# RTCartist/Neuromorphic-Spatiotemporal-Optical-Flow

Measured on AMD Instinct MI355X. Metric: 1080p frame-pairs/sec (Farneback, HIP), higher is better.
Workload: dtype f32

## Files before the change

### include/nsof.h

```cpp
#ifndef NSOF_H
#define NSOF_H

#include <stddef.h>
#include <stdint.h>

#ifdef __cplusplus
extern "C" {
#endif

#define NSOF_ABI_VERSION 3

typedef enum nsof_status {
    NSOF_OK = 0,
    NSOF_EINVAL = -1,
    NSOF_ESHAPE = -2,
    NSOF_EDEVICE = -3,
    NSOF_ENOMEM = -4,
    NSOF_EUNSUPPORTED = -5
} nsof_status;

typedef struct nsof_ctx nsof_ctx;

int nsof_create(int device, nsof_ctx** out);
void nsof_destroy(nsof_ctx* ctx);
const char* nsof_last_error(const nsof_ctx* ctx);
int nsof_abi_version(void);
int nsof_set_stream(nsof_ctx* ctx, void* hip_stream);
int nsof_synchronize(nsof_ctx* ctx);
enum { NSOF_OPT_POLYEXP_F32 = 1, NSOF_OPT_EXACT_ROWSUMS = 2, NSOF_OPT_ROW_BANDS = 3, NSOF_OPT_PYR_FMA = 4,
       NSOF_OPT_SMALL_BATCH_JOBS = 5, NSOF_OPT_DEBUG_FAULT = 100 };
int nsof_set_option(nsof_ctx* ctx, int option, int value);
int nsof_get_option(const nsof_ctx* ctx, int option, int* value);

enum { NSOF_USE_INITIAL_FLOW = 4, NSOF_FARNEBACK_GAUSSIAN = 256 };

typedef enum nsof_pixel_type {
    NSOF_PIXEL_U8 = 0,
    NSOF_PIXEL_F32 = 1,
    NSOF_PIXEL_U16 = 2,
    NSOF_PIXEL_S16 = 3,
} nsof_pixel_type;

int nsof_farneback_px(nsof_ctx* ctx, int pixel_type,
                      const void* prev, ptrdiff_t prev_stride,
                      const void* next, ptrdiff_t next_stride,
                      int width, int height,
                      float* flow, ptrdiff_t flow_stride,
                      double pyr_scale, int levels, int winsize, int iterations,
                      int poly_n, double poly_sigma, int flags);
int nsof_farneback_u8(nsof_ctx* ctx,
                      const uint8_t* prev, ptrdiff_t prev_stride,
                      const uint8_t* next, ptrdiff_t next_stride,
                      int width, int height,
                      float* flow, ptrdiff_t flow_stride,
                      double pyr_scale, int levels, int winsize, int iterations,
                      int poly_n, double poly_sigma, int flags);
int nsof_farneback_f32(nsof_ctx* ctx,
                       const float* prev, ptrdiff_t prev_stride,
                       const float* next, ptrdiff_t next_stride,
                       int width, int height,
                       float* flow, ptrdiff_t flow_stride,
                       double pyr_scale, int levels, int winsize, int iterations,
                       int poly_n, double poly_sigma, int flags);

int nsof_farneback_px_batch_dev(nsof_ctx* ctx, int pixel_type, int n_pairs,
                                const void* d_prev, const void* d_next,
                                ptrdiff_t row_stride, ptrdiff_t pair_stride,
                                int width, int height, float* d_flow,
                                double pyr_scale, int levels, int winsize, int iterations,
                                int poly_n, double poly_sigma, int flags);
int nsof_farneback_u8_batch_dev(nsof_ctx* ctx, int n_pairs,
                                const uint8_t* d_prev, const uint8_t* d_next,
                                ptrdiff_t row_stride, ptrdiff_t pair_stride,
                                int width, int height, float* d_flow,
                                double pyr_scale, int levels, int winsize, int iterations,
                                int poly_n, double poly_sigma, int flags);
int nsof_farneback_f32_batch_dev(nsof_ctx* ctx, int n_pairs,
                                 const float* d_prev, const float* d_next,
                                 ptrdiff_t row_stride, ptrdiff_t pair_stride,
                                 int width, int height, float* d_flow,
                                 double pyr_scale, int levels, int winsize, int iterations,
                                 int poly_n, double poly_sigma, int flags);

int nsof_farneback_px_sequence_dev(nsof_ctx* ctx, int pixel_type, int n_frames, const void* d_frames,
                                   ptrdiff_t row_stride, ptrdiff_t frame_stride,
                                   int width, int height, float* d_flow,
                                   double pyr_scale, int levels, int winsize, int iterations,
                                   int poly_n, double poly_sigma, int flags);
int nsof_farneback_u8_sequence_dev(nsof_ctx* ctx, int n_frames, const uint8_t* d_frames,
                                   ptrdiff_t row_stride, ptrdiff_t frame_stride,
                                   int width, int height, float* d_flow,
                                   double pyr_scale, int levels, int winsize, int iterations,
                                   int poly_n, double poly_sigma, int flags);
int nsof_farneback_f32_sequence_dev(nsof_ctx* ctx, int n_frames, const float* d_frames,
                                    ptrdiff_t row_stride, ptrdiff_t frame_stride,
                                    int width, int height, float* d_flow,
                                    double pyr_scale, int levels, int winsize, int iterations,
                                    int poly_n, double poly_sigma, int flags);

typedef struct nsof_pair_desc_px {
    const void* prev;
    ptrdiff_t prev_stride;
    const void* next;
    ptrdiff_t next_stride;
    int width, height;
    float* flow;
    ptrdiff_t flow_stride;
} nsof_pair_desc_px;
typedef struct nsof_pair_desc {
    const uint8_t* prev;
    ptrdiff_t prev_stride;
    const uint8_t* next;
    ptrdiff_t next_stride;
    int width, height;
    float* flow;
    ptrdiff_t flow_stride;
} nsof_pair_desc;
typedef struct nsof_pair_desc_f32 {
    const float* prev;
    ptrdiff_t prev_stride;
    const float* next;
    ptrdiff_t next_stride;
    int width, height;
    float* flow;
    ptrdiff_t flow_stride;
} nsof_pair_desc_f32;

int nsof_farneback_px_batch(nsof_ctx* ctx, int pixel_type, int n_pairs, const nsof_pair_desc_px* pairs,
                            double pyr_scale, int levels, int winsize, int iterations,
                            int poly_n, double poly_sigma, int flags);
int nsof_farneback_u8_batch(nsof_ctx* ctx, int n_pairs, const nsof_pair_desc* pairs,
                            double pyr_scale, int levels, int winsize, int iterations,
                            int poly_n, double poly_sigma, int flags);
int nsof_farneback_f32_batch(nsof_ctx* ctx, int n_pairs, const nsof_pair_desc_f32* pairs,
                             double pyr_scale, int levels, int winsize, int iterations,
                             int poly_n, double poly_sigma, int flags);

int nsof_farneback_px_batch_desc_dev(nsof_ctx* ctx, int pixel_type, int n_pairs, const nsof_pair_desc_px* pairs,
                                     double pyr_scale, int levels, int winsize, int iterations,
                                     int poly_n, double poly_sigma, int flags);
int nsof_farneback_u8_batch_desc_dev(nsof_ctx* ctx, int n_pairs, const nsof_pair_desc* pairs,
                                     double pyr_scale, int levels, int winsize, int iterations,
                                     int poly_n, double poly_sigma, int flags);
int nsof_farneback_f32_batch_desc_dev(nsof_ctx* ctx, int n_pairs, const nsof_pair_desc_f32* pairs,
                                      double pyr_scale, int levels, int winsize, int iterations,
                                      int poly_n, double poly_sigma, int flags);

int nsof_farneback_px_roi_sequence_dev(nsof_ctx* ctx, int pixel_type, int n_frames, const void* d_frames,
                                       ptrdiff_t row_stride, ptrdiff_t frame_stride, int width, int height,
                                       const int32_t* d_counts, const int32_t* d_rects, int max_rects, float* d_flows,
                                       double pyr_scale, int levels, int winsize, int iterations, int poly_n,
                                       double poly_sigma, int flags, int gate_frame, long long* n_calls,
                                       long long* n_pixels);
int nsof_farneback_u8_roi_sequence_dev(nsof_ctx* ctx, int n_frames, const uint8_t* d_frames, ptrdiff_t row_stride,
                                       ptrdiff_t frame_stride, int width, int height, const int32_t* d_counts,
                                       const int32_t* d_rects, int max_rects, float* d_flows, double pyr_scale, int levels,
                                       int winsize, int iterations, int poly_n, double poly_sigma, int flags,
                                       int gate_frame, long long* n_calls, long long* n_pixels);
int nsof_farneback_f32_roi_sequence_dev(nsof_ctx* ctx, int n_frames, const float* d_frames, ptrdiff_t row_stride,
                                        ptrdiff_t frame_stride, int width, int height, const int32_t* d_counts,
                                        const int32_t* d_rects, int max_rects, float* d_flows, double pyr_scale, int levels,
                                        int winsize, int iterations, int poly_n, double poly_sigma, int flags,
                                        int gate_frame, long long* n_calls, long long* n_pixels);
void* nsof_host_alloc(size_t bytes);
void nsof_host_free(void* p);

int nsof_farneback_effective_levels(int width, int height, double pyr_scale, int levels);
int nsof_farneback_level_size(int width, int height, double pyr_scale, int level,
                              int* level_width, int* level_height, int* blur_ksize, double* blur_sigma);

int nsof_stage_pyr_level_px(nsof_ctx* ctx, int pixel_type, int n_img, const void* d_src, ptrdiff_t row_stride,
                            ptrdiff_t img_stride, int width, int height, double pyr_scale, int level, float* d_out);
int nsof_stage_pyr_level(nsof_ctx* ctx, int n_img, const uint8_t* d_src, ptrdiff_t row_stride,
                         ptrdiff_t img_stride, int width, int height, double pyr_scale, int level, float* d_out);
int nsof_stage_pyr_level_f32(nsof_ctx* ctx, int n_img, const float* d_src, ptrdiff_t row_stride,
                             ptrdiff_t img_stride, int width, int height, double pyr_scale, int level, float* d_out);
int nsof_stage_polyexp(nsof_ctx* ctx, int n_img, const float* d_img, int width, int height,
                       int poly_n, double poly_sigma, float* d_R);
int nsof_stage_recip(nsof_ctx* ctx, long long n, const double* d_x, double* d_out, double* d_ieee);
int nsof_stage_update_matrices(nsof_ctx* ctx, int n_pairs, const float* d_R, const float* d_flow,
                               int width, int height, float* d_M);
int nsof_stage_blur_solve(nsof_ctx* ctx, int n_pairs, const float* d_M, int width, int height,
                          int winsize, float* d_flow);
int nsof_stage_gauss_blur_solve(nsof_ctx* ctx, int n_pairs, const float* d_M, int width, int height,
                                int winsize, float* d_flow);
int nsof_stage_iterate(nsof_ctx* ctx, int n_pairs, const float* d_R, const float* d_flow_in, int width, int height,
                       int winsize, float* d_flow_out);
int nsof_stage_iterate_upsample(nsof_ctx* ctx, int n_pairs, const float* d_R, const float* d_coarse_flow,
                                int src_w, int src_h, int width, int height, int winsize, double pyr_scale,
                                float* d_flow_out);
int nsof_stage_flow_upsample(nsof_ctx* ctx, int n_pairs, const float* d_src, int src_w, int src_h,
                             float* d_dst, int dst_w, int dst_h, double pyr_scale);

typedef enum nsof_kernel_id {
    NSOF_K_PREP = 0,
    NSOF_K_POLYEXP = 1,
    NSOF_K_UPSAMPLE = 2,
    NSOF_K_UPDMAT = 3,
    NSOF_K_BLUR = 4,
    NSOF_K_ACCUM = 5,
    NSOF_K_ITERATE = 6,
    NSOF_K_SEGMENT = 7,
    NSOF_K_MORPH = 8,
    NSOF_K_REMAP = 9,
    NSOF_K_SSIM = 10,
    NSOF_K_COUNT = 11
} nsof_kernel_id;
int nsof_prof_enable(nsof_ctx* ctx, unsigned mask);
int nsof_prof_collect(nsof_ctx* ctx, int kernel_id, double* total_ms, long long* launches);
const char* nsof_kernel_name(int kernel_id);

typedef struct nsof_accum nsof_accum;

int nsof_accum_create(nsof_ctx* ctx, int height, int width, int scheme, int polarity_split,
                      float active_v, float silent_v, nsof_accum** out);
typedef struct nsof_accum_params {
    double alphaoff, alphaon, voff, von, koff, kon, son, soff, bon, boff, Ron, Roff, wini;
    double dt;
    int64_t refractory_us;
} nsof_accum_params;
void nsof_accum_default_params(nsof_accum_params* out);
int nsof_accum_create_p(nsof_ctx* ctx, int height, int width, int scheme, int polarity_split, float active_v, float silent_v,
                        const nsof_accum_params* params, nsof_accum** out);
int nsof_accum_get_params(const nsof_accum* acc, nsof_accum_params* out);
enum {
    NSOF_ACCUM_KEY_ALPHAOFF = 0, NSOF_ACCUM_KEY_ALPHAON, NSOF_ACCUM_KEY_VOFF, NSOF_ACCUM_KEY_VON, NSOF_ACCUM_KEY_KOFF,
    NSOF_ACCUM_KEY_KON, NSOF_ACCUM_KEY_SON, NSOF_ACCUM_KEY_SOFF, NSOF_ACCUM_KEY_BON, NSOF_ACCUM_KEY_BOFF, NSOF_ACCUM_KEY_RON,
    NSOF_ACCUM_KEY_ROFF, NSOF_ACCUM_KEY_WINI, NSOF_ACCUM_KEY_COUNT
};
int nsof_accum_set_param_maps(nsof_accum* acc, int n_maps, const int* keys, const float* const* maps);
int nsof_accum_read_param_map(nsof_accum* acc, int key, float* out);
int nsof_accum_param_map_mask(const nsof_accum* acc, unsigned* mask);
void nsof_accum_destroy(nsof_accum* acc);
int nsof_accum_set_dense(nsof_accum* acc, int force_dense);
int nsof_accum_set_event_threshold(nsof_accum* acc, int theta);
int nsof_accum_get_event_threshold(const nsof_accum* acc, int* theta);
int nsof_accum_reset(nsof_accum* acc);
int nsof_accum_step_events(nsof_accum* acc, const int16_t* x, const int16_t* y, const int8_t* p,
                           const int64_t* t, const int64_t* slice_bounds, int64_t n_slices,
                           int64_t snap_every);
int nsof_accum_set_events(nsof_accum* acc, const int16_t* x, const int16_t* y, const int8_t* p,
                          const int64_t* t, const int64_t* slice_bounds, int64_t n_slices);
int nsof_accum_run(nsof_accum* acc, int64_t first_slice, int64_t n_slices, int64_t snap_every);
int nsof_accum_set_slice_times(nsof_accum* acc, const int64_t* t_first, const int64_t* t_last, int64_t n_slices);
enum { NSOF_SURFACE_CURRENT = 0, NSOF_SURFACE_STATE = 1 };
int nsof_accum_surface_u8_dev(nsof_accum* acc, int which, int mode, uint8_t* d_out, ptrdiff_t row_stride);
int nsof_accum_surface_f32_dev(nsof_accum* acc, int which, int mode, float* d_out, ptrdiff_t row_stride_bytes);
int nsof_accum_run_surface(nsof_accum* a, int64_t first_slice, int64_t n_slices, int which, int mode, uint8_t* d_out,
                           ptrdiff_t row_stride);
int nsof_accum_run_frames(nsof_accum* acc, int64_t first_slice, int64_t n_frames, int64_t every, int which, int mode,
                          uint8_t* d_frames, ptrdiff_t row_stride, ptrdiff_t frame_stride);
int nsof_accum_set_frames_path(nsof_accum* acc, int path);
int nsof_accum_read_state(nsof_accum* acc, int which, float* w_out, int64_t* next_ok_out, int64_t* slice_counter);
int nsof_accum_write_state(nsof_accum* acc, int which, const float* w_in, const int64_t* next_ok_in,
                           int64_t slice_counter);
int nsof_accum_update_state_dev(nsof_ctx* ctx, const float* d_w, const float* d_V, float* d_out, size_t n);
int nsof_accum_update_state_p_dev(nsof_ctx* ctx, const nsof_accum_params* params, const float* d_w, const float* d_V,
                                  float* d_out, size_t n);
int nsof_accum_bincount_2d(nsof_ctx* ctx, const int16_t* x, const int16_t* y, size_t n, int height, int width,
                           int32_t* counts_out);
int nsof_accum_resistance_dev(nsof_ctx* ctx, const float* d_w, float* d_out, size_t n);
int nsof_accum_resistance_p_dev(nsof_ctx* ctx, const nsof_accum_params* params, const float* d_w, float* d_out, size_t n);
int nsof_accum_read_w(nsof_accum* acc, int which, float* w_out);
int nsof_accum_read_resistance(nsof_accum* acc, int which, float* r_out);
int64_t nsof_accum_snapshot_count(const nsof_accum* acc);
int nsof_accum_read_snapshots(nsof_accum* acc, int which, float* out, int64_t max_count);
int nsof_accum_block_current(nsof_accum* acc, int which, int64_t snapshot, int memsize, double v_ds, double* out);
int nsof_accum_block_current_dev(nsof_accum* acc, int which, int64_t snapshot, int memsize, double v_ds, double* d_out);
int nsof_accum_frames_f64(nsof_ctx* ctx, const double* imgs, int n_frames, int height, int width, double dt,
                          int n_sub_steps, double th1, double th2, double* w_out, double* res_out);
int nsof_accum_frames_f64_p(nsof_ctx* ctx, const double* imgs, int n_frames, int height, int width, double dt,
                            int n_sub_steps, double th1, double th2, const nsof_accum_params* params, double* w_out,
                            double* res_out);
int nsof_accum_frames_f64_dev(nsof_ctx* ctx, const double* d_imgs, int n_frames, int height, int width, double dt,
                              int n_sub_steps, double th1, double th2, double v_ds, double* d_w, double* d_res,
                              double* d_current);
int nsof_accum_frames_f64_p_dev(nsof_ctx* ctx, const double* d_imgs, int n_frames, int height, int width, double dt,
                                int n_sub_steps, double th1, double th2, double v_ds, const nsof_accum_params* params,
                                double* d_w, double* d_res, double* d_current);
int nsof_accum_frames_f64_maps_dev(nsof_ctx* ctx, const double* d_imgs, int n_frames, int height, int width, double dt,
                                   int n_sub_steps, double th1, double th2, double v_ds, const nsof_accum_params* params,
                                   int n_trials, int n_maps, const int* keys, const double* const* planes,
                                   const int* plane_trials, double* d_w, double* d_res, double* d_current);
int nsof_accum_frames_f64_maps(nsof_ctx* ctx, const double* imgs, int n_frames, int height, int width, double dt,
                               int n_sub_steps, double th1, double th2, const nsof_accum_params* params, int n_trials,
                               int n_maps, const int* keys, const double* const* planes, const int* plane_trials,
                               double* w_out, double* res_out);
int nsof_accum_trials_dev(nsof_ctx* ctx, int height, int width, int scheme, int polarity_split, float active_v, float silent_v,
                          const nsof_accum_params* params, int theta, const int16_t* x, const int16_t* y, const int8_t* p,
                          const int64_t* t, const int64_t* slice_bounds, int64_t n_slices, int64_t snap_every, int memsize,
                          double v_ds, int n_trials, int n_maps, const int* keys, const float* const* planes,
                          const int* plane_trials, float* d_w, float* d_resistance, double* d_block_current);
int nsof_frames_compress_u8_dev(nsof_ctx* ctx, int n_frames, const uint8_t* d_frames, ptrdiff_t row_stride,
                                ptrdiff_t frame_stride, int width, int height, int out_w, int out_h, const double* wts_y,
                                const int32_t* ind_y, int taps_y, const double* wts_x, const int32_t* ind_x, int taps_x,
                                double* d_out);
int nsof_lanczos3_contributions(int in_len, int out_len, double* wts, int32_t* ind, int cap_taps, int* taps);
int64_t nsof_accum_slice_bounds(const int64_t* t, int64_t n, int64_t slice_us, int64_t* idx, int64_t cap);

int nsof_roi_from_surface(const double* current, int rows, int cols, int frame_w, int frame_h, int memsize, int thres,
                          int extend_left, int extend_right, int extend_upper, int extend_lower, int connectivity,
                          int flag, int* rects, int max_rects);

int nsof_roi_from_surface_dev(nsof_ctx* ctx, const double* d_current, int n_maps, size_t map_stride, int rows, int cols,
                              int frame_w, int frame_h, int memsize, int thres, int extend_left, int extend_right,
                              int extend_upper, int extend_lower, int connectivity, int flag, int max_rects, int* d_counts,
                              int* d_rects, unsigned char* d_gray);
int nsof_gate_stats_dev(nsof_ctx* ctx, const double* d_current, const double* d_nominal, int n_trials, int n_frames, int rows,
                        int cols, int thres, int* d_counts, int* d_flips);

enum { NSOF_MORPH_RECT = 0, NSOF_MORPH_CROSS = 1, NSOF_MORPH_ELLIPSE = 2 };
enum { NSOF_MORPH_ERODE = 0, NSOF_MORPH_DILATE = 1 };
int nsof_structuring_element(int shape, int kw, int kh, uint8_t* out);
int nsof_morph_binary_u8_dev(nsof_ctx* ctx, int op, const uint8_t* d_src, ptrdiff_t src_stride, int width,
                             int height, const uint8_t* elem, int kw, int kh, int anchor_x, int anchor_y,
                             int iterations, uint8_t* d_dst, ptrdiff_t dst_stride);
int nsof_motion_mask_dev(nsof_ctx* ctx, const float* d_flow, ptrdiff_t flow_stride_floats, int width, int height,
                         double thresh, int ksize, int iterations, uint8_t* d_mask, ptrdiff_t mask_stride);
int nsof_motion_mask_sequence_dev(nsof_ctx* ctx, int n_pairs, const float* d_flows, int width, int height,
                                  const int32_t* box_counts, const int32_t* boxes, double thresh, int ksize,
                                  int iterations, uint8_t* d_masks);
int nsof_pixel_accuracy_u8_batch_dev(nsof_ctx* ctx, int n, const uint8_t* d_masks, const uint8_t* d_gt,
                                     ptrdiff_t gt_row_stride, ptrdiff_t gt_frame_stride, int width, int height,
                                     double* d_out);
int nsof_motion_mask(nsof_ctx* ctx, const float* flow, ptrdiff_t flow_stride_bytes, int width, int height,
                     double thresh, int ksize, int iterations, uint8_t* mask, ptrdiff_t mask_stride);

enum { NSOF_BORDER_CONSTANT = 0, NSOF_BORDER_REPLICATE = 1 };
int nsof_gray_u8_dev(nsof_ctx* ctx, const uint8_t* d_src, ptrdiff_t src_stride, int width, int height, int bgr_weights,
                     uint8_t* d_dst, ptrdiff_t dst_stride);
int nsof_remap_linear_u8_dev(nsof_ctx* ctx, const uint8_t* d_src, ptrdiff_t src_stride, int src_w, int src_h,
                             int channels, const float* d_map_x, ptrdiff_t map_x_stride_floats,
                             const float* d_map_y, ptrdiff_t map_y_stride_floats, int dst_w, int dst_h,
                             int border_mode, int border_value, uint8_t* d_dst, ptrdiff_t dst_stride);
int nsof_predict_warp_u8_dev(nsof_ctx* ctx, const uint8_t* d_frame, ptrdiff_t frame_stride, int width, int height,
                             int channels, const float* d_flow, ptrdiff_t flow_stride_floats, int sign,
                             int x0, int y0, int x1, int y1, int border_mode, uint8_t* d_out, ptrdiff_t out_stride);
int nsof_predict_warp_u8(nsof_ctx* ctx, const uint8_t* frame, ptrdiff_t frame_stride, int width, int height,
                         int channels, const float* flow_crop, ptrdiff_t flow_stride_bytes, int sign,
                         int x0, int y0, int x1, int y1, int border_mode, uint8_t* out, ptrdiff_t out_stride);
int nsof_ssim_u8_dev(nsof_ctx* ctx, const uint8_t* d_a, ptrdiff_t a_stride, int a_pixel_step, const uint8_t* d_b,
                     ptrdiff_t b_stride, int b_pixel_step, int width, int height, double data_range,
                     double* ssim_out);
int nsof_ssim_u8(nsof_ctx* ctx, const uint8_t* a, ptrdiff_t a_stride, int a_pixel_step, const uint8_t* b,
                 ptrdiff_t b_stride, int b_pixel_step, int width, int height, double data_range, double* ssim_out);
int nsof_predict_sequence_u8_dev(nsof_ctx* ctx, int n_pairs, const uint8_t* d_frames, ptrdiff_t row_stride,
                                 ptrdiff_t frame_stride, int width, int height, const float* d_flows, int sign,
                                 const int32_t* d_counts, const int32_t* d_rects, int n_maps, int max_rects,
                                 int gate_frame, int merge_padding, int border_mode, uint8_t* d_out);
int nsof_ssim_u8_batch_dev(nsof_ctx* ctx, int n, const uint8_t* d_a, ptrdiff_t a_stride, ptrdiff_t a_item_stride,
                           int a_pixel_step, const uint8_t* d_b, ptrdiff_t b_stride, ptrdiff_t b_item_stride,
                           int b_pixel_step, int width, int height, double data_range, double* d_out);
int nsof_flow_to_image_dev(nsof_ctx* ctx, int n, const float* d_flows, ptrdiff_t row_stride_floats,
                           ptrdiff_t item_stride_floats, int width, int height, int sign, double clip_flow,
                           double max_flow, int convert_to_bgr, uint8_t* d_out, ptrdiff_t out_row_stride,
                           ptrdiff_t out_item_stride, float* d_norms);

#ifdef __cplusplus
}
#endif
#endif
```

### neuromorphic-spatiotemporal-optical-flow_amd/csrc/farneback_driver.hip

```cpp
#include <cstdlib>
#include <cstring>

#include "nsof_internal.h"

struct Carve {
    std::vector<size_t> offI, offR;
    size_t szI = 0, szR = 0, szS = 0, szM = 0, szV = 0;
    char* base = nullptr;
    size_t total() const { return szI + szR + szS + szM + szV; }
    float* level_I(int k) const { return (float*)(base + offI[k]); }
    float* level_R(int k) const { return (float*)(base + szI + offR[k]); }
    float* S() const { return (float*)(base + szI + szR); }
    float* M() const { return (float*)(base + szI + szR + szS); }
    double* V() const { return (double*)(base + szI + szR + szS + szM); }
};
static Carve farneback_carve(size_t B, bool sequence, int width, int height, double pyr_scale, int L, bool lat,
                             nsof_iter_form form)
{
    Carve c;
    c.offI.assign(L + 1, 0);
    c.offR.assign(L + 1, 0);
    const size_t n0 = (size_t)width * height;
    const size_t n_img = sequence ? B + 1 : 2 * B;
    for (int k = 0; k <= (lat ? L : 0); k++) {
        int wk, hk;
        nsof_farneback_level_size(width, height, pyr_scale, k, &wk, &hk, nullptr, nullptr);
        c.offI[k] = c.szI;
        c.offR[k] = c.szR;
        c.szI += align_up(n_img * (size_t)wk * hk * 4, 256);
        c.szR += align_up(n_img * 5 * (size_t)wk * hk * 4, 256);
    }
    c.szS = align_up(B * n0 * 8, 256);
    const bool M = form != NSOF_ITER_FAST && form != NSOF_ITER_EXACT;
    const bool V = form == NSOF_ITER_UNFUSED_EXACT || form == NSOF_ITER_EXACT_LAT;
    c.szM = M ? align_up(B * 5 * n0 * 4, 256) : 0;
    c.szV = V ? align_up(B * 5 * n0 * 8, 256) : 0;
    return c;
}

struct Run {
    nsof_ctx* ctx;
    const nsof_fb_frames& f;
    const nsof_fb_params& p;
    int L;
    nsof_iter_form form;
    bool lat;
    Carve cv;
    size_t B, n_img;
    int arrays, n_first;
    nsof_poly_taps ptaps;
    float* Ifused[4] = {nullptr, nullptr, nullptr, nullptr};
};

static int level_images(const Run& r, int k, int wk, int hk, const nsof_blur_taps& bt)
{
    const nsof_fb_frames& f = r.f;
    float* Rk = r.cv.level_R(k);
    if (k >= 1 && k <= 3 && r.Ifused[k]) return nsof_launch_polyexp(r.ctx, (int)r.n_img, r.Ifused[k], wk, hk, r.ptaps, Rk);
    if (k == 0 && nsof_level0_from_frames(r.ctx, f.src, bt) && f.width >= 2 && f.height >= 2 && wk == f.width && hk == f.height)
        return nsof_launch_polyexp_frames(r.ctx, (int)r.n_img, f.prev, r.arrays == 1 ? f.prev : f.next, r.n_first, f.row_stride,
                                          f.pair_stride, f.width, f.height, r.ptaps, bt.k[1], bt.k[2], Rk, f.src);
    float* I = r.cv.level_I(k);
    for (int i = 0; i < r.arrays; i++)
        if (int rc = nsof_launch_prep(r.ctx, r.n_first, i == 0 ? f.prev : f.next, f.row_stride, f.pair_stride, f.width, f.height, wk,
                                      hk, bt, I + (size_t)i * r.B * wk * hk, f.src))
            return rc;
    return nsof_launch_polyexp(r.ctx, (int)r.n_img, I, wk, hk, r.ptaps, Rk);
}

static int side_stream_images(const Run& r)
{
    nsof_ctx* ctx = r.ctx;
    const int L = r.L;
    if (!ctx->side) NSOF_HIP(ctx, hipStreamCreateWithFlags(&ctx->side, hipStreamNonBlocking));
    while (ctx->ov_events.size() < (size_t)(L + 2)) {
        hipEvent_t ev;
        NSOF_HIP(ctx, hipEventCreateWithFlags(&ev, hipEventDisableTiming));
        ctx->ov_events.push_back(ev);
    }
    const hipStream_t mainS = ctx->stream, sideS = ctx->side;
    struct Restore { nsof_ctx* cx; hipStream_t saved; ~Restore() { cx->stream = saved; } } restore{ctx, mainS};
    NSOF_HIP(ctx, hipEventRecord(ctx->ov_events[L + 1], mainS));
    NSOF_HIP(ctx, hipStreamWaitEvent(sideS, ctx->ov_events[L + 1], 0));
    for (int k = L; k >= 0; k--) {
        int wk, hk;
        nsof_blur_taps bt;
        if (int rc = nsof_level_geom(ctx, r.f.width, r.f.height, r.p.pyr_scale, k, &wk, &hk, &bt)) return rc;
        ctx->stream = k == L ? mainS : sideS;
        if (int rc = level_images(r, k, wk, hk, bt)) return rc;
        if (k < L) NSOF_HIP(ctx, hipEventRecord(ctx->ov_events[k], sideS));
    }
    return NSOF_OK;
}

static int three_level_images(Run& r)
{
    const nsof_fb_frames& f = r.f;
    nsof_blur_taps bt3[3];
    size_t nk3[3];
    for (int k = 1; k <= 3; k++) {
        int wk, hk;
        if (nsof_level_geom(nullptr, f.width, f.height, r.p.pyr_scale, k, &wk, &hk, &bt3[k - 1]) != 0 ||
            wk * (1 << k) != f.width || hk * (1 << k) != f.height)
            return NSOF_OK;
        nk3[k - 1] = (size_t)wk * hk;
    }
    float* dI = r.cv.level_I(0);
    float* I3[3] = {dI, dI + r.n_img * nk3[0], dI + r.n_img * (nk3[0] + nk3[1])};
    int rc = NSOF_OK;
    for (size_t i = 0; i < (size_t)r.arrays && rc == NSOF_OK; i++) {
        float* I3i[3] = {I3[0] + i * r.B * nk3[0], I3[1] + i * r.B * nk3[1], I3[2] + i * r.B * nk3[2]};
        rc = nsof_launch_prep_decim3(r.ctx, r.n_first, i == 0 ? f.prev : f.next, f.row_stride, f.pair_stride, f.width, f.height, bt3,
                                     I3i, f.src);
    }
    if (rc == NSOF_OK)
        for (int k = 1; k <= 3; k++) r.Ifused[k] = I3[k - 1];
    return rc == NSOF_EUNSUPPORTED ? NSOF_OK : rc;
}

static int iterate_level(const Run& r, int k, int wk, int hk, float* const fb[2], int* cur)
{
    nsof_ctx* ctx = r.ctx;
    const int n_pairs = r.f.n_pairs, winsize = r.p.winsize;
    const size_t nk = (size_t)wk * hk;
    const float* R0 = r.cv.level_R(k);
    const float* R1 = R0 + (r.f.sequence ? (size_t)1 : r.B) * 5 * nk;
    float* dM = r.cv.M();
    double* dV = r.cv.V();
    for (int it = 0; it < r.p.iterations; it++) {
        int rc;
        if (nsof_form_fused(r.form)) {
            float* in = fb[*cur];
            float* out = fb[*cur ^= 1];
            if (r.form == NSOF_ITER_EXACT_LAT) rc = nsof_launch_iterate_lat(ctx, n_pairs, R0, R1, 5 * nk, in, out, wk, hk, winsize, dM, dV);
            else if (r.form == NSOF_ITER_EXACT) rc = nsof_launch_iterate_x(ctx, n_pairs, R0, R1, 5 * nk, in, out, wk, hk, winsize);
            else rc = nsof_launch_iterate(ctx, n_pairs, R0, R1, 5 * nk, in, out, wk, hk, winsize);
        } else {
            float* flow = fb[*cur];
            if ((rc = nsof_launch_update_matrices(ctx, n_pairs, R0, R1, 5 * nk, flow, wk, hk, dM))) return rc;
            if (r.form == NSOF_ITER_UNFUSED_GAUSS) rc = nsof_launch_gauss_blur_solve(ctx, n_pairs, dM, wk, hk, winsize, flow);
            else if (r.form == NSOF_ITER_UNFUSED_EXACT) rc = nsof_launch_blur_solve_exact(ctx, n_pairs, dM, wk, hk, winsize, dV, flow);
            else rc = nsof_launch_blur_solve(ctx, n_pairs, dM, wk, hk, winsize, flow);
        }
        if (rc) return rc;
    }
    return NSOF_OK;
}

static int run_levels(Run& r, float* d_flow)
{
    nsof_ctx* ctx = r.ctx;
    const nsof_fb_frames& f = r.f;
    const int L = r.L, iterations = r.p.iterations;
    int rc = nsof_host_poly_taps(r.p.poly_n, r.p.poly_sigma, &r.ptaps);
    if (rc) return nsof_set_error(ctx, rc, "poly taps");
    if ((rc = ctx->ws.reserve(ctx, r.cv.total()))) return rc;
    r.cv.base = (char*)ctx->ws.p;
    float* const fb[2] = {d_flow, r.cv.S()};
    const int flips = nsof_form_fused(r.form) ? L * (1 + iterations) + iterations : L;
    int cur = flips & 1;

    const hipStream_t mainS = ctx->stream;
    if (r.lat) rc = side_stream_images(r);
    else if (L == 3) rc = three_level_images(r);
    if (rc) return rc;

    int pw = 0, ph = 0;
    for (int k = L; k >= 0; k--) {
        int wk, hk;
        nsof_blur_taps btaps;
        if ((rc = nsof_level_geom(ctx, f.width, f.height, r.p.pyr_scale, k, &wk, &hk, &btaps))) return rc;
        if (k == L) {
            NSOF_HIP(ctx, hipMemsetAsync(fb[cur], 0, r.B * wk * hk * 8, mainS));
        } else {
            if ((rc = nsof_launch_flow_upsample(ctx, f.n_pairs, fb[cur], pw, ph, fb[cur ^ 1], wk, hk, (float)(1. / r.p.pyr_scale))))
                return rc;
            cur ^= 1;
        }
        if (!r.lat) {
            if ((rc = level_images(r, k, wk, hk, btaps))) return rc;
        } else if (k < L) {
            NSOF_HIP(ctx, hipStreamWaitEvent(mainS, ctx->ov_events[k], 0));
        }
        if ((rc = iterate_level(r, k, wk, hk, fb, &cur))) return rc;
        pw = wk;
        ph = hk;
    }
    if (fb[cur] != d_flow)
        NSOF_HIP(ctx, hipMemcpyAsync(d_flow, fb[cur], r.B * f.width * f.height * 8, hipMemcpyDeviceToDevice, mainS));
    return NSOF_OK;
}

static int pairs_per_run(Run& r, size_t* fit)
{
    nsof_ctx* ctx = r.ctx;
    auto carve = [&](size_t b) { return farneback_carve(b, r.f.sequence, r.f.width, r.f.height, r.p.pyr_scale, r.L, r.lat, r.form); };
    size_t n = (size_t)r.f.n_pairs;
    if (r.form == NSOF_ITER_UNFUSED_EXACT && n > 64) n = 64;
    r.cv = carve(n);
    if (r.cv.total() > ctx->ws.cap) {
        size_t free_b = 0, total_b = 0;
        NSOF_HIP(ctx, hipMemGetInfo(&free_b, &total_b));
        const size_t budget = (size_t)((double)(free_b + ctx->ws.cap) * 0.92);
        size_t lo = 0, hi = n;
        while (lo < hi) {
            const size_t mid = (lo + hi + 1) / 2;
            if (carve(mid).total() <= budget) lo = mid;
            else hi = mid - 1;
        }
        n = lo;
    }
    if (const char* e = getenv("NSOF_MAX_PAIRS")) {
        const long v = atol(e);
        if (v >= 1 && (size_t)v < n) n = (size_t)v;
    }
    if (n < 1) n = 1;
    if (n > 32767) n = 32767;
    *fit = n;
    return NSOF_OK;
}

int nsof_farneback_core(nsof_ctx* ctx, const nsof_fb_frames& frames, float* d_flow, const nsof_fb_params& p)
{
    if (!ctx) return NSOF_EINVAL;
    nsof_fb_frames f = frames;
    if (f.sequence) f.next = f.prev;
    if (!f.prev || !f.next || !d_flow || f.n_pairs < 1) return nsof_set_error(ctx, NSOF_EINVAL, "null buffer or n_pairs<1");
    int rc = nsof_check_farneback_params(ctx, f.width, f.height, p);
    if (rc) return rc;
    if (!nsof_row_stride_holds(f.row_stride, f.width, f.src))
        return nsof_set_error(ctx, NSOF_EINVAL, "row_stride < width * %d", nsof_src_bytes(f.src));
    NSOF_HIP(ctx, hipSetDevice(ctx->device));
    const nsof_iter_form form = nsof_iterate_form(ctx, p.winsize, f.width, f.height, p.iterations,
                                                  f.n_pairs * nsof_iterate_jobs(f.width, f.height), p.flags);
    if (form == NSOF_ITER_UNFUSED_EXACT && f.sequence) {
        f.sequence = false;
        f.next = f.prev + f.pair_stride;
    }
    const int L = nsof_farneback_effective_levels(f.width, f.height, p.pyr_scale, p.levels);
    Run r{ctx, f, p, L, form, form == NSOF_ITER_EXACT_LAT && L >= 1};
    size_t fit;
    if ((rc = pairs_per_run(r, &fit))) return rc;
    if ((size_t)f.n_pairs > fit) {
        nsof_fb_frames c = f;
        for (int i = 0; i < f.n_pairs; i += (int)fit) {
            c.n_pairs = f.n_pairs - i < (int)fit ? f.n_pairs - i : (int)fit;
            c.prev = f.prev + (ptrdiff_t)i * f.pair_stride;
            c.next = f.next + (ptrdiff_t)i * f.pair_stride;
            if ((rc = nsof_farneback_core(ctx, c, d_flow + (size_t)i * f.width * f.height * 2, p))) return rc;
        }
        return NSOF_OK;
    }
    r.B = (size_t)f.n_pairs;
    r.n_img = f.sequence ? r.B + 1 : 2 * r.B;
    r.arrays = f.sequence || f.next == f.prev + (ptrdiff_t)f.n_pairs * f.pair_stride ? 1 : 2;
    r.n_first = r.arrays == 1 ? (int)r.n_img : f.n_pairs;
    return run_levels(r, d_flow);
}

extern "C" int nsof_farneback_px_batch_dev(nsof_ctx* ctx, int pixel_type, int n_pairs, const void* d_prev, const void* d_next,
                                           ptrdiff_t row_stride, ptrdiff_t pair_stride, int width, int height, float* d_flow,
                                           double pyr_scale, int levels, int winsize, int iterations, int poly_n,
                                           double poly_sigma, int flags)
{
    if (int rc = nsof_check_typed(ctx, pixel_type)) return rc;
    if (!d_prev || !d_next || !d_flow) return nsof_set_error(ctx, NSOF_EINVAL, "null buffer");
    int rc = nsof_check_frame_layout(ctx, pixel_type, d_prev, row_stride, pair_stride, width, "d_prev");
    if (rc == NSOF_OK) rc = nsof_check_frame_layout(ctx, pixel_type, d_next, row_stride, pair_stride, width, "d_next");
    if (rc) return rc;
    return nsof_farneback_core(ctx, {false, n_pairs, (const uint8_t*)d_prev, (const uint8_t*)d_next, row_stride, pair_stride, width,
                                     height, pixel_type},
                               d_flow, {pyr_scale, levels, winsize, iterations, poly_n, poly_sigma, flags});
}

extern "C" int nsof_farneback_px_sequence_dev(nsof_ctx* ctx, int pixel_type, int n_frames, const void* d_frames,
                                              ptrdiff_t row_stride, ptrdiff_t frame_stride, int width, int height,
                                              float* d_flow, double pyr_scale, int levels, int winsize, int iterations,
                                              int poly_n, double poly_sigma, int flags)
{
    if (int rc = nsof_check_typed(ctx, pixel_type)) return rc;
    if (n_frames < 2) return nsof_set_error(ctx, NSOF_EINVAL, "a sequence needs at least 2 frames");
    if (!d_frames || !d_flow) return nsof_set_error(ctx, NSOF_EINVAL, "null buffer");
    if (int rc = nsof_check_frame_layout(ctx, pixel_type, d_frames, row_stride, frame_stride, width, "d_frames")) return rc;
    return nsof_farneback_core(ctx, {true, n_frames - 1, (const uint8_t*)d_frames, nullptr, row_stride, frame_stride, width, height,
                                     pixel_type},
                               d_flow, {pyr_scale, levels, winsize, iterations, poly_n, poly_sigma, flags});
}

extern "C" int nsof_farneback_px(nsof_ctx* ctx, int src, const void* prev, ptrdiff_t prev_stride, const void* next,
                                 ptrdiff_t next_stride, int width, int height, float* flow, ptrdiff_t flow_stride,
                                 double pyr_scale, int levels, int winsize, int iterations, int poly_n,
                                 double poly_sigma, int flags)
{
    if (int rc = nsof_check_typed(ctx, src)) return rc;
    const nsof_fb_params p{pyr_scale, levels, winsize, iterations, poly_n, poly_sigma, flags};
    if (!prev || !next || !flow) return nsof_set_error(ctx, NSOF_EINVAL, "null image pointer");
    int rc = nsof_check_farneback_params(ctx, width, height, p);
    if (rc) return rc;
    if ((rc = nsof_check_frame_layout(ctx, src, prev, prev_stride, 0, width, "prev")) ||
        (rc = nsof_check_frame_layout(ctx, src, next, next_stride, 0, width, "next")))
        return rc;
    if (flow_stride < (ptrdiff_t)(width * 8)) return nsof_set_error(ctx, NSOF_EINVAL, "flow_stride < width*8");
    NSOF_HIP(ctx, hipSetDevice(ctx->device));
    const size_t n0 = (size_t)width * height, pitch = (size_t)width * nsof_src_bytes(src);
    const size_t szU = align_up(pitch * height, 256), szF = align_up(n0 * 8, 256);
    if ((rc = ctx->stage.reserve(ctx, 2 * szU + szF)) || (rc = ctx->hstage.reserve(ctx, 2 * szU + szF))) return rc;
    char* hP = (char*)ctx->hstage.p;
    char* hN = hP + szU;
    float* hF = (float*)(hN + szU);
    uint8_t* dP = (uint8_t*)ctx->stage.p;
    uint8_t* dN = dP + szU;
    float* dFl = (float*)(dN + szU);
    const bool in_dense = prev_stride == (ptrdiff_t)pitch && next_stride == (ptrdiff_t)pitch;
    const bool out_dense = flow_stride == (ptrdiff_t)width * 8;
    if (in_dense) {
        NSOF_HIP(ctx, hipMemcpyAsync(dP, prev, pitch * height, hipMemcpyHostToDevice, ctx->stream));
        NSOF_HIP(ctx, hipMemcpyAsync(dN, next, pitch * height, hipMemcpyHostToDevice, ctx->stream));
    } else {
        for (int y = 0; y < height; y++) {
            memcpy(hP + (size_t)y * pitch, (const char*)prev + (ptrdiff_t)y * prev_stride, pitch);
            memcpy(hN + (size_t)y * pitch, (const char*)next + (ptrdiff_t)y * next_stride, pitch);
        }
        NSOF_HIP(ctx, hipMemcpyAsync(dP, hP, 2 * szU, hipMemcpyHostToDevice, ctx->stream));
    }
    if ((rc = nsof_farneback_core(ctx, {false, 1, dP, dN, (ptrdiff_t)pitch, (ptrdiff_t)szU, width, height, src}, dFl, p))) return rc;
    NSOF_HIP(ctx, hipMemcpyAsync(out_dense ? flow : hF, dFl, n0 * 8, hipMemcpyDeviceToHost, ctx->stream));
    if ((rc = nsof_stream_sync_checked(ctx))) return rc;
    if (!out_dense)
        for (int y = 0; y < height; y++)
            memcpy((char*)flow + (ptrdiff_t)y * flow_stride, hF + (size_t)y * width * 2, (size_t)width * 8);
    return NSOF_OK;
}

extern "C" int nsof_farneback_u8(nsof_ctx* ctx, const uint8_t* prev, ptrdiff_t prev_stride, const uint8_t* next,
                                 ptrdiff_t next_stride, int width, int height, float* flow, ptrdiff_t flow_stride,
                                 double pyr_scale, int levels, int winsize, int iterations, int poly_n,
                                 double poly_sigma, int flags)
{
    return nsof_farneback_px(ctx, NSOF_PIXEL_U8, prev, prev_stride, next, next_stride, width, height, flow, flow_stride,
                             pyr_scale, levels, winsize, iterations, poly_n, poly_sigma, flags);
}

extern "C" int nsof_farneback_f32(nsof_ctx* ctx, const float* prev, ptrdiff_t prev_stride, const float* next,
                                  ptrdiff_t next_stride, int width, int height, float* flow, ptrdiff_t flow_stride,
                                  double pyr_scale, int levels, int winsize, int iterations, int poly_n,
                                  double poly_sigma, int flags)
{
    return nsof_farneback_px(ctx, NSOF_PIXEL_F32, prev, prev_stride, next, next_stride, width, height, flow, flow_stride,
                             pyr_scale, levels, winsize, iterations, poly_n, poly_sigma, flags);
}

extern "C" int nsof_farneback_u8_batch_dev(nsof_ctx* ctx, int n_pairs, const uint8_t* d_prev, const uint8_t* d_next,
                                           ptrdiff_t row_stride, ptrdiff_t pair_stride, int width, int height,
                                           float* d_flow, double pyr_scale, int levels, int winsize, int iterations,
                                           int poly_n, double poly_sigma, int flags)
{
    return nsof_farneback_px_batch_dev(ctx, NSOF_PIXEL_U8, n_pairs, d_prev, d_next, row_stride, pair_stride, width, height,
                                       d_flow, pyr_scale, levels, winsize, iterations, poly_n, poly_sigma, flags);
}

extern "C" int nsof_farneback_f32_batch_dev(nsof_ctx* ctx, int n_pairs, const float* d_prev, const float* d_next,
                                            ptrdiff_t row_stride, ptrdiff_t pair_stride, int width, int height,
                                            float* d_flow, double pyr_scale, int levels, int winsize, int iterations,
                                            int poly_n, double poly_sigma, int flags)
{
    return nsof_farneback_px_batch_dev(ctx, NSOF_PIXEL_F32, n_pairs, d_prev, d_next, row_stride, pair_stride, width, height,
                                       d_flow, pyr_scale, levels, winsize, iterations, poly_n, poly_sigma, flags);
}

extern "C" int nsof_farneback_u8_sequence_dev(nsof_ctx* ctx, int n_frames, const uint8_t* d_frames,
                                              ptrdiff_t row_stride, ptrdiff_t frame_stride, int width, int height,
                                              float* d_flow, double pyr_scale, int levels, int winsize,
                                              int iterations, int poly_n, double poly_sigma, int flags)
{
    return nsof_farneback_px_sequence_dev(ctx, NSOF_PIXEL_U8, n_frames, d_frames, row_stride, frame_stride, width, height,
                                          d_flow, pyr_scale, levels, winsize, iterations, poly_n, poly_sigma, flags);
}

extern "C" int nsof_farneback_f32_sequence_dev(nsof_ctx* ctx, int n_frames, const float* d_frames,
                                               ptrdiff_t row_stride, ptrdiff_t frame_stride, int width, int height,
                                               float* d_flow, double pyr_scale, int levels, int winsize,
                                               int iterations, int poly_n, double poly_sigma, int flags)
{
    return nsof_farneback_px_sequence_dev(ctx, NSOF_PIXEL_F32, n_frames, d_frames, row_stride, frame_stride, width, height,
                                          d_flow, pyr_scale, levels, winsize, iterations, poly_n, poly_sigma, flags);
}
```

### neuromorphic-spatiotemporal-optical-flow_amd/csrc/farneback_iterate_x.hip

```cpp
#include "iterate_common.h"

namespace {

typedef __attribute__((address_space(1))) unsigned long long gu64;
typedef __attribute__((address_space(1))) unsigned gu32;
typedef __attribute__((address_space(3))) int lds_int;

__device__ __forceinline__ unsigned xcc_id() { return __builtin_amdgcn_s_getreg(20 | (0 << 6) | (3 << 11)) & 7u; }

template <int MH>
struct XGeom {
    static constexpr int COLS = 208, NCW = 3, RB = 4;
    static constexpr int RL = 2 * MH + 1 + 2 * RB;
    static constexpr int HALO = 2 * MH + 1;
    static constexpr int SW = NCW * 64;
    static_assert(SW + HALO <= COLS && SW % 8 == 0, "strip geometry");
    static constexpr int NB = COLS / 64, REM = COLS % 64;
    static_assert(REM == 16, "the remainder wave maps 4 rows x 16 columns onto its 64 lanes");
    static constexpr int SEG0 = 96, SEG1 = SW - SEG0;
    static_assert(SEG0 % 8 == 0 && SEG1 % 8 == 0 && SEG0 >= SEG1 && SEG1 > 0, "segments: whole 8-column blocks, the left one not shorter");
    static constexpr int SVW = SW + 2;
    static constexpr int WAVES = NCW + 1 + 2 * NB + 1 + 1;
    static constexpr int THREADS = 64 * WAVES;
    static constexpr int CQ = 1, IOQ = 1;
    static constexpr size_t SV1_BYTES = sizeof(double) * 4 * 5 * SVW;
    static constexpr size_t SV_BYTES = 2 * SV1_BYTES;
    static constexpr size_t VI_BYTES = sizeof(double) * 2 * 4 * 5 * MH;
    static constexpr size_t JOB_BYTES = 16;
    static constexpr size_t CB_BYTES = sizeof(double) * 2 * 2 * 20;
    static constexpr size_t RING4_BYTES = sizeof(float) * 4 * RL * COLS, RING1_BYTES = sizeof(float) * RL * COLS;
    static constexpr size_t SMEM = SV_BYTES + VI_BYTES + JOB_BYTES + CB_BYTES + RING4_BYTES + RING1_BYTES;
};

struct XRing {
    float4* q;
    float* c;
    int cols;
    __device__ __forceinline__ void put(int slot, int col, const float (&M)[5]) const
    {
        q[slot * cols + col] = make_float4(M[0], M[1], M[2], M[3]);
        c[slot * cols + col] = M[4];
    }
    __device__ __forceinline__ void get(int slot, int col, float (&M)[5]) const
    {
        const float4 v = q[slot * cols + col];
        M[0] = v.x; M[1] = v.y; M[2] = v.z; M[3] = v.w;
        M[4] = c[slot * cols + col];
    }
};

constexpr unsigned X_SPIN_LIMIT = 1u << 21;

template <int MH>
__device__ __forceinline__ void x_produce(RowIn& in, float2& dd, float2& fl, const XRing& ring, const Planes& R0,
                                          const Planes& R1, const FlowSrc& F, int W, int H, int xc, int col, int i)
{
    constexpr int RL = XGeom<MH>::RL;
    float Mn[5];
    matrix_from(in, dd.x, dd.y, xc, min(i, H - 1), W, H, Mn);
    ring.put((i + MH + 1) % RL, col, Mn);
    issue_row(in, R0, R1, W, H, xc, min(i + 8, H - 1), fl);
    dd = fl;
    fl = F.fetch(min(i + 16, H - 1));
}

template <int MH>
__device__ __forceinline__ void x_rows_above(const XRing& ring, const Planes& R0, const Planes& R1, const FlowSrc& F,
                                             int W, int H, int xc, int col)
{
    float2 fl[MH];
#pragma unroll
    for (int i = 0; i < MH; i++) fl[i] = F.fetch(min(i, H - 1));
    constexpr int GRP = 4;
#pragma unroll
    for (int g0 = 0; g0 < MH; g0 += GRP) {
        RowIn t[GRP];
#pragma unroll
        for (int k = 0; k < GRP; k++)
            if (g0 + k < MH) issue_row(t[k], R0, R1, W, H, xc, min(g0 + k, H - 1), fl[g0 + k]);
#pragma unroll
        for (int k = 0; k < GRP; k++)
            if (g0 + k < MH) {
                float Mi[5];
                matrix_from(t[k], fl[g0 + k].x, fl[g0 + k].y, xc, min(g0 + k, H - 1), W, H, Mi);
                if (g0 + k == 0) {
#pragma unroll
                    for (int j = 0; j <= MH + 1; j++) ring.put(j, col, Mi);
                } else {
                    ring.put(g0 + k + MH + 1, col, Mi);
                }
            }
    }
}

template <int MH, int GP>
__device__ __forceinline__ void x_producer_loop(const XRing& ring, const Planes& R0, const Planes& R1,
                                                const FlowSrc& F, int W, int H, int xc, int col, int nimg)
{
    if constexpr (GP == 0) x_rows_above<MH>(ring, R0, R1, F, W, H, xc, col);
    RowIn in[2][2];
    float2 dd[2][2], fl[2][2];
#pragma unroll
    for (int ts = 0; ts < 2; ts++)
#pragma unroll
        for (int rr = 0; rr < 2; rr++) {
            const int r = min(4 * ts + MH + 2 * GP + rr, H - 1);
            dd[ts][rr] = F.fetch(r);
            issue_row(in[ts][rr], R0, R1, W, H, xc, r, dd[ts][rr]);
        }
#pragma unroll
    for (int ts = 0; ts < 2; ts++)
#pragma unroll
        for (int rr = 0; rr < 2; rr++) fl[ts][rr] = F.fetch(min(4 * (ts + 2) + MH + 2 * GP + rr, H - 1));
    auto step = [&](auto tsc, int t) {
        constexpr int TS = decltype(tsc)::value;
        x_produce<MH>(in[TS][0], dd[TS][0], fl[TS][0], ring, R0, R1, F, W, H, xc, col, 4 * t + MH + 2 * GP);
        x_produce<MH>(in[TS][1], dd[TS][1], fl[TS][1], ring, R0, R1, F, W, H, xc, col, 4 * t + MH + 2 * GP + 1);
    };
    step(std::integral_constant<int, 0>{}, 0);
    __syncthreads();
    step(std::integral_constant<int, 1>{}, 1);
    __syncthreads();
    int t = 0;
    for (; t < nimg; t += 2) {
        step(std::integral_constant<int, 0>{}, t + 2);
        __syncthreads();
        step(std::integral_constant<int, 1>{}, t + 3);
        __syncthreads();
    }
    if (t == nimg) {
        step(std::integral_constant<int, 0>{}, t + 2);
        __syncthreads();
    }
}

template <int MH, int Q0, int NQ>
__device__ __forceinline__ void x_solve_rows(const double* sv, volatile lds_int* flag, float2* Fout, size_t fpitch, int W, int H,
                                             int x0, int nimg, double scale, int lane, int t)
{
    using G = XGeom<MH>;
    constexpr int SVW = G::SVW, NBLK = G::SW / 64;
    double g[NBLK][NQ][5];
    int us[NBLK];
#pragma unroll
    for (int b = 0; b < NBLK; b++) {
        const int col = b * 64 + lane;
        const int u = t - 1 - (col >= G::SEG0 ? 1 : 0);
        us[b] = (u >= 0 && u < nimg && x0 + col < W) ? u : -1;
        const double* p = sv + (u & 1) * (G::SV1_BYTES / sizeof(double)) + col;
#pragma unroll
        for (int q = 0; q < NQ; q++)
#pragma unroll
            for (int c = 0; c < 5; c++) g[b][q][c] = p[((q + Q0) * 5 + c) * SVW];
    }
    asm volatile("s_waitcnt lgkmcnt(0)" ::: "memory");
    if (lane == 0) *flag = t + 1;
#pragma unroll
    for (int b = 0; b < NBLK; b++) {
        if (us[b] < 0) continue;
        const int x = x0 + b * 64 + lane;
#pragma unroll
        for (int q = 0; q < NQ; q++) {
            const int yo = 4 * us[b] + q + Q0;
            const float2 o = nsof_flow_solve(g[b][q][0], g[b][q][1], g[b][q][2], g[b][q][3], g[b][q][4], scale);
            if (yo < H) nsof_store_stream2(reinterpret_cast<float*>(Fout + (size_t)yo * fpitch + x), o.x, o.y);
        }
    }
}

template <int MH>
__device__ __forceinline__ void x_remainder_loop(const XRing& ring, double* cb, const Planes& R0, const Planes& R1,
                                                 const FlowSrc& F, int W, int H, int xc, int col, int r, int nimg,
                                                 gu64* cin, gu64* cout, unsigned epoch, gu32* err, const double* sv,
                                                 volatile lds_int* ioflag, float2* Fout, size_t fpitch, int x0, double scale)
{
    const int lane = threadIdx.x & 63;
    const bool io = lane < 20;
    const int l = io ? lane : 0;
    unsigned long long g0 = 0, g1 = 0;
    auto carry_load = [&](int s) {
        const gu64* q = cin + 40 * s + 2 * l;
        asm volatile("global_load_dwordx2 %0, %2, off sc1\n\tglobal_load_dwordx2 %1, %2, off offset:8 sc1"
                     : "=&v"(g0), "=&v"(g1) : "v"(q) : "memory");
    };
    auto fetch_issue = [&](int s) {
        if (!cin || !io) return;
        carry_load(s);
    };
    bool dead = false;
    auto fetch_finish = [&](int s) {
        if (!cin || !io) return;
        asm volatile("s_waitcnt vmcnt(9)" : "+v"(g0), "+v"(g1) : : "memory");
        for (unsigned spins = 0; !dead; spins++) {
            if (__all((unsigned)(g0 >> 32) == epoch && (unsigned)(g1 >> 32) == epoch)) break;
            if (spins > X_SPIN_LIMIT ||
                ((spins & 255u) == 255u && __hip_atomic_load(err, __ATOMIC_RELAXED, __HIP_MEMORY_SCOPE_AGENT) != 0u)) {
                if (lane == 0) __hip_atomic_fetch_or(err, 1u, __ATOMIC_RELAXED, __HIP_MEMORY_SCOPE_AGENT);
                dead = true;
                break;
            }
            __builtin_amdgcn_s_sleep(8);
            carry_load(s);
            asm volatile("s_waitcnt vmcnt(0)" : "+v"(g0), "+v"(g1) : : "memory");
        }
        cb[40 + (s & 1) * 20 + l] = __hiloint2double((int)(unsigned)g1, (int)(unsigned)g0);
    };
    auto publish = [&](int s) {
        if (!cout || !io) return;
        const double S = cb[(s & 1) * 20 + l];
        const unsigned long long tag = (unsigned long long)epoch << 32;
        __hip_atomic_store(cout + 40 * s + 2 * l, tag | (unsigned)__double2loint(S), __ATOMIC_RELAXED, __HIP_MEMORY_SCOPE_AGENT);
        __hip_atomic_store(cout + 40 * s + 2 * l + 1, tag | (unsigned)__double2hiint(S), __ATOMIC_RELAXED, __HIP_MEMORY_SCOPE_AGENT);
    };
    if (r == 0) x_rows_above<MH>(ring, R0, R1, F, W, H, xc, col);
    RowIn in[2];
    float2 dd[2], fl[2];
#pragma unroll
    for (int ts = 0; ts < 2; ts++) {
        const int y = min(4 * ts + MH + r, H - 1);
        dd[ts] = F.fetch(y);
        issue_row(in[ts], R0, R1, W, H, xc, y, dd[ts]);
    }
#pragma unroll
    for (int ts = 0; ts < 2; ts++) fl[ts] = F.fetch(min(4 * (ts + 2) + MH + r, H - 1));
    x_produce<MH>(in[0], dd[0], fl[0], ring, R0, R1, F, W, H, xc, col, MH + r);
    __syncthreads();
    fetch_issue(0);
    x_produce<MH>(in[1], dd[1], fl[1], ring, R0, R1, F, W, H, xc, col, 4 + MH + r);
    fetch_finish(0);
    __syncthreads();
    auto window = [&](auto tsc, int t) {
        constexpr int TS = decltype(tsc)::value;
        if (t >= 2) publish(t - 2);
        if (t + 1 < nimg) fetch_issue(t + 1);
        x_produce<MH>(in[TS], dd[TS], fl[TS], ring, R0, R1, F, W, H, xc, col, 4 * (t + 2) + MH + r);
        x_solve_rows<MH, XGeom<MH>::CQ, XGeom<MH>::IOQ>(sv, ioflag, Fout, fpitch, W, H, x0, nimg, scale, lane, t);
        if (t + 1 < nimg) fetch_finish(t + 1);
        __syncthreads();
    };
    int t = 0;
    for (; t < nimg; t += 2) {
        window(std::integral_constant<int, 0>{}, t);
        window(std::integral_constant<int, 1>{}, t + 1);
    }
    if (t == nimg) window(std::integral_constant<int, 0>{}, t);
    publish(nimg - 1);
    x_solve_rows<MH, XGeom<MH>::CQ, XGeom<MH>::IOQ>(sv, ioflag, Fout, fpitch, W, H, x0, nimg, scale, lane, nimg + 1);
}

template <int MH>
__device__ __forceinline__ void x_consumer_loop(const XRing& ring, double* sv, double* vinit, volatile lds_int* sflag, float2* Fout,
                                                size_t fpitch, int W, int H, int x0, int j, int nimg, double scale, bool strip0)
{
    using G = XGeom<MH>;
    constexpr int RL = G::RL, SVW = G::SVW, HALO = G::HALO;
    const int rb = j, ra = j + HALO;
    const int vik = j == 0 ? 0 : j - MH - 1;
    const bool vi_thread = strip0 && (j == 0 || (j >= MH + 2 && j <= 2 * MH));
    __syncthreads();
    double va[5], vb[5];
    {
        float a0[5], b0[5];
        ring.get(MH + 1, ra, a0);
        ring.get(MH + 1, rb, b0);
#pragma unroll
        for (int c = 0; c < 5; c++) {
            va[c] = (double)(a0[c] * (float)(MH + 2));
            vb[c] = (double)(b0[c] * (float)(MH + 2));
        }
#pragma unroll
        for (int i = 1; i < MH; i++) {
            ring.get(i + MH + 1, ra, a0);
            ring.get(i + MH + 1, rb, b0);
#pragma unroll
            for (int c = 0; c < 5; c++) {
                va[c] += (double)a0[c];
                vb[c] += (double)b0[c];
            }
        }
    }
    int slot_new = (2 * MH + 1) % RL;
    int slot_old = 0;
    const int x = x0 + j;
    const int lag = j >= G::SEG0 ? 1 : 0;
    double D[2][4][5];
    auto column_sums = [&](auto pc, int s) {
        constexpr int P = decltype(pc)::value;
#pragma unroll
        for (int q = 0; q < 4; q++) {
            float na[5], oa[5], nb[5], ob[5];
            ring.get(slot_new, ra, na);
            ring.get(slot_old, ra, oa);
            ring.get(slot_new, rb, nb);
            ring.get(slot_old, rb, ob);
#pragma unroll
            for (int c = 0; c < 5; c++) {
                const float da = na[c] - oa[c];
                const float db = nb[c] - ob[c];
                va[c] += (double)da;
                vb[c] += (double)db;
                D[P][q][c] = va[c] - vb[c];
            }
            if (vi_thread) {
#pragma unroll
                for (int c = 0; c < 5; c++) vinit[(((s & 1) * 4 + q) * 5 + c) * MH + vik] = vb[c];
            }
            slot_new = slot_new + 1 == RL ? 0 : slot_new + 1;
            slot_old = slot_old + 1 == RL ? 0 : slot_old + 1;
        }
    };
    auto publish = [&](auto pc, int p) {
        constexpr int P = decltype(pc)::value;
        if (p < 0 || p >= nimg) return;
        double* svj = sv + (p & 1) * (G::SV1_BYTES / sizeof(double)) + j;
#pragma unroll
        for (int q = 0; q < 4; q++)
#pragma unroll
            for (int c = 0; c < 5; c++) svj[(q * 5 + c) * SVW] = D[P][q][c];
    };
    column_sums(std::integral_constant<int, 0>{}, 0);
    if (!lag) publish(std::integral_constant<int, 0>{}, 0);
    __syncthreads();
    auto window = [&](auto pc, int t) {
        constexpr int P = decltype(pc)::value;
        const int u = t - 1 - lag;
        if (u >= 0 && u < nimg && x < W) {
            const double* svj = sv + (u & 1) * (G::SV1_BYTES / sizeof(double)) + j;
#pragma unroll
            for (int q = 0; q < G::CQ; q++) {
                const int yo = 4 * u + q;
                const double* s = svj + q * 5 * SVW;
                const float2 o = nsof_flow_solve(s[0], s[SVW], s[2 * SVW], s[3 * SVW], s[4 * SVW], scale);
                if (yo < H) nsof_store_stream2(reinterpret_cast<float*>(Fout + (size_t)yo * fpitch + x), o.x, o.y);
            }
        }
        if (t == nimg + 1) return;
        if (t + 1 < nimg) column_sums(std::integral_constant<int, P ^ 1>{}, t + 1);
        for (int spin = 0; (sflag[0] < t + 1 || sflag[1] < t + 1) && spin < (1 << 22); spin++)
            __builtin_amdgcn_s_sleep(1);
        if (lag) publish(std::integral_constant<int, P>{}, t);
        else publish(std::integral_constant<int, P ^ 1>{}, t + 1);
        __syncthreads();
    };
    for (int t = 0; t <= nimg + 1; t += 2) {
        window(std::integral_constant<int, 0>{}, t);
        if (t + 1 > nimg + 1) break;
        window(std::integral_constant<int, 1>{}, t + 1);
    }
}

template <int MH>
__device__ __forceinline__ void x_solver_loop(const double* sv, volatile lds_int* sflag, float2* Fout, size_t fpitch, int W, int H,
                                              int x0, int nimg, double scale, int lane)
{
    using G = XGeom<MH>;
    __syncthreads();
    __syncthreads();
    for (int t = 0; t <= nimg + 1; t++) {
        x_solve_rows<MH, G::CQ + G::IOQ, 4 - G::CQ - G::IOQ>(sv, sflag, Fout, fpitch, W, H, x0, nimg, scale, lane, t);
        if (t <= nimg) __syncthreads();
    }
}

template <int MH>
__device__ __forceinline__ void x_scanner_loop(double* sv, const double* vinit, double* cb, bool has_left, int nimg, int ncols,
                                               int lane)
{
    using G = XGeom<MH>;
    constexpr int SVW = G::SVW;
    typedef double d2 __attribute__((ext_vector_type(2)));
    const int seg = lane >= 20 ? 1 : 0;
    const int l = lane < 40 ? lane - 20 * seg : 0;
    double Smid = 0.;
    __syncthreads();
    __builtin_amdgcn_s_setprio(3);
    __syncthreads();
    for (int t = 0; t <= nimg; t++) {
        const int step = t - seg;
        const double Sleft = __shfl(Smid, lane >= 20 ? lane - 20 : lane);
        d2* row = reinterpret_cast<d2*>(sv + (step & 1) * (G::SV1_BYTES / sizeof(double)) + l * SVW + seg * G::SEG0);
        if (lane < 40 && step >= 0 && step < nimg) {
            double S;
            if (seg) {
                S = Sleft;
            } else if (has_left) {
                S = cb[40 + (step & 1) * 20 + l];
            } else {
                const double* vi = vinit + ((step & 1) * 20 + l) * MH;
                S = vi[0] * (double)(MH + 2);
#pragma unroll
                for (int k = 1; k < MH; k++) S += vi[k];
            }
            auto scan_blocks = [&](int b0, int nb) {
                unsigned a = (unsigned)(size_t)(__attribute__((address_space(3))) char*)(row + 4 * b0);
                int nrem = nb - 1;
                asm volatile(
                "ds_read_b128 v[64:67], %[a]\n\t"
                "ds_read_b128 v[68:71], %[a] offset:16\n\t"
                "ds_read_b128 v[72:75], %[a] offset:32\n\t"
                "ds_read_b128 v[76:79], %[a] offset:48\n\t"
                "ds_read_b128 v[80:83], %[a] offset:64\n\t"
                "ds_read_b128 v[84:87], %[a] offset:80\n\t"
                "ds_read_b128 v[88:91], %[a] offset:96\n\t"
                "ds_read_b128 v[92:95], %[a] offset:112\n\t"
                "s_waitcnt lgkmcnt(7)\n\t"
                "v_add_f64 v[64:65], %[S], v[64:65]\n\t"
                "v_add_f64 v[66:67], v[66:67], v[64:65]\n\t"
                "s_waitcnt lgkmcnt(6)\n\t"
                "v_add_f64 v[68:69], v[66:67], v[68:69]\n\t"
                "v_add_f64 v[70:71], v[70:71], v[68:69]\n\t"
                "s_waitcnt lgkmcnt(5)\n\t"
                "v_add_f64 v[72:73], v[70:71], v[72:73]\n\t"
                "v_add_f64 v[74:75], v[74:75], v[72:73]\n\t"
                "s_waitcnt lgkmcnt(4)\n\t"
                "v_add_f64 v[76:77], v[74:75], v[76:77]\n\t"
                "v_add_f64 v[78:79], v[78:79], v[76:77]\n\t"
                "s_nop 1\n\t"
                "ds_write_b128 %[a], v[64:67]\n\t"
                "ds_write_b128 %[a], v[68:71] offset:16\n\t"
                "ds_write_b128 %[a], v[72:75] offset:32\n\t"
                "ds_write_b128 %[a], v[76:79] offset:48\n\t"
                "s_cmp_lt_i32 %[n], 2\n\t"
                "s_cbranch_scc1 .Lxs_tail%=\n"
                ".Lxs_loop%=:\n\t"
                "s_waitcnt lgkmcnt(7)\n\t"
                "v_add_f64 v[80:81], v[78:79], v[80:81]\n\t"
                "ds_read_b128 v[64:67], %[a] offset:128\n\t"
                "ds_read_b128 v[68:71], %[a] offset:144\n\t"
                "ds_read_b128 v[72:75], %[a] offset:160\n\t"
                "ds_read_b128 v[76:79], %[a] offset:176\n\t"
                "v_add_f64 v[82:83], v[82:83], v[80:81]\n\t"
                "s_waitcnt lgkmcnt(10)\n\t"
                "v_add_f64 v[84:85], v[82:83], v[84:85]\n\t"
                "v_add_f64 v[86:87], v[86:87], v[84:85]\n\t"
                "s_waitcnt lgkmcnt(9)\n\t"
                "v_add_f64 v[88:89], v[86:87], v[88:89]\n\t"
                "v_add_f64 v[90:91], v[90:91], v[88:89]\n\t"
                "s_waitcnt lgkmcnt(8)\n\t"
                "v_add_f64 v[92:93], v[90:91], v[92:93]\n\t"
                "v_add_f64 v[94:95], v[94:95], v[92:93]\n\t"
                "s_nop 1\n\t"
                "ds_write_b128 %[a], v[80:83] offset:64\n\t"
                "ds_write_b128 %[a], v[84:87] offset:80\n\t"
                "ds_write_b128 %[a], v[88:91] offset:96\n\t"
                "ds_write_b128 %[a], v[92:95] offset:112\n\t"
                "s_waitcnt lgkmcnt(7)\n\t"
                "v_add_f64 v[64:65], v[94:95], v[64:65]\n\t"
                "ds_read_b128 v[80:83], %[a] offset:192\n\t"
                "ds_read_b128 v[84:87], %[a] offset:208\n\t"
                "ds_read_b128 v[88:91], %[a] offset:224\n\t"
                "ds_read_b128 v[92:95], %[a] offset:240\n\t"
                "v_add_f64 v[66:67], v[66:67], v[64:65]\n\t"
                "s_waitcnt lgkmcnt(10)\n\t"
                "v_add_f64 v[68:69], v[66:67], v[68:69]\n\t"
                "v_add_f64 v[70:71], v[70:71], v[68:69]\n\t"
                "s_waitcnt lgkmcnt(9)\n\t"
                "v_add_f64 v[72:73], v[70:71], v[72:73]\n\t"
                "v_add_f64 v[74:75], v[74:75], v[72:73]\n\t"
                "s_waitcnt lgkmcnt(8)\n\t"
                "v_add_f64 v[76:77], v[74:75], v[76:77]\n\t"
                "v_add_f64 v[78:79], v[78:79], v[76:77]\n\t"
                "s_nop 1\n\t"
                "ds_write_b128 %[a], v[64:67] offset:128\n\t"
                "ds_write_b128 %[a], v[68:71] offset:144\n\t"
                "ds_write_b128 %[a], v[72:75] offset:160\n\t"
                "ds_write_b128 %[a], v[76:79] offset:176\n\t"
                "v_add_u32 %[a], 128, %[a]\n\t"
                "s_sub_i32 %[n], %[n], 2\n\t"
                "s_cmp_ge_i32 %[n], 2\n\t"
                "s_cbranch_scc1 .Lxs_loop%=\n"
                ".Lxs_tail%=:\n\t"
                "s_cmp_lt_i32 %[n], 1\n\t"
                "s_cbranch_scc1 .Lxs_done%=\n\t"
                "s_waitcnt lgkmcnt(4)\n\t"
                "v_add_f64 v[80:81], v[78:79], v[80:81]\n\t"
                "v_add_f64 v[82:83], v[82:83], v[80:81]\n\t"
                "s_waitcnt lgkmcnt(4)\n\t"
                "v_add_f64 v[84:85], v[82:83], v[84:85]\n\t"
                "v_add_f64 v[86:87], v[86:87], v[84:85]\n\t"
                "s_waitcnt lgkmcnt(4)\n\t"
                "v_add_f64 v[88:89], v[86:87], v[88:89]\n\t"
                "v_add_f64 v[90:91], v[90:91], v[88:89]\n\t"
                "s_waitcnt lgkmcnt(4)\n\t"
                "v_add_f64 v[92:93], v[90:91], v[92:93]\n\t"
                "v_add_f64 v[94:95], v[94:95], v[92:93]\n\t"
                "s_nop 1\n\t"
                "ds_write_b128 %[a], v[80:83] offset:64\n\t"
                "ds_write_b128 %[a], v[84:87] offset:80\n\t"
                "ds_write_b128 %[a], v[88:91] offset:96\n\t"
                "ds_write_b128 %[a], v[92:95] offset:112\n\t"
                "v_mov_b64 v[78:79], v[94:95]\n"
                ".Lxs_done%=:\n\t"
                "v_mov_b64 %[S], v[78:79]\n\t"
                "s_waitcnt lgkmcnt(0)\n\t"
                    : [S] "+v"(S), [a] "+v"(a), [n] "+s"(nrem)
                    :
                    : "memory", "scc", "v64", "v65", "v66", "v67", "v68", "v69", "v70", "v71", "v72", "v73", "v74", "v75", "v76", "v77", "v78", "v79", "v80", "v81", "v82", "v83", "v84", "v85", "v86", "v87", "v88", "v89", "v90", "v91", "v92", "v93", "v94", "v95");
            };
            const int nb0 = ncols >> 3, nba = nb0 < G::SEG1 / 8 ? nb0 : G::SEG1 / 8;
            scan_blocks(0, nba);
            if (nb0 > nba && !seg) scan_blocks(nba, nb0 - nba);
            if (seg) cb[(step & 1) * 20 + l] = S;
            else Smid = S;
        }
        __syncthreads();
    }
}

template <int MH, bool HET>
__global__ __launch_bounds__((XGeom<MH>::THREADS)) void k_iterate_x(
    const float* __restrict__ R0b, const float* __restrict__ R1b, size_t pair_stride, const float* __restrict__ flow_in,
    float* __restrict__ flow_out, int W, int H, int block_size, const nsof_het_item* __restrict__ items, int het_final,
    int n, int nstrips, unsigned long long* carry, unsigned* tickets, unsigned epoch, unsigned* err, int fault,
    const unsigned* __restrict__ xjobs)
{
    using G = XGeom<MH>;
    constexpr int SW = G::SW, COLS = G::COLS;
    extern __shared__ __attribute__((aligned(16))) unsigned char smem_x[];
    double* sv = reinterpret_cast<double*>(smem_x);
    double* vinit = reinterpret_cast<double*>(smem_x + G::SV_BYTES);
    int* job = reinterpret_cast<int*>(smem_x + G::SV_BYTES + G::VI_BYTES);
    double* cb = reinterpret_cast<double*>(smem_x + G::SV_BYTES + G::VI_BYTES + G::JOB_BYTES);
    XRing ring;
    ring.q = reinterpret_cast<float4*>(smem_x + G::SV_BYTES + G::VI_BYTES + G::JOB_BYTES + G::CB_BYTES);
    ring.c = reinterpret_cast<float*>(smem_x + G::SV_BYTES + G::VI_BYTES + G::JOB_BYTES + G::CB_BYTES + G::RING4_BYTES);
    ring.cols = COLS;
    const int tid = threadIdx.x;
    if (tid == 0) {
        const unsigned share = HET ? 0u : (unsigned)((n + 7) / 8) * (unsigned)nstrips;
        unsigned k = xcc_id();
        unsigned lim = HET ? xjobs[k] : share;
        unsigned i = __hip_atomic_fetch_add(tickets + 32 * k, 1u, __ATOMIC_RELAXED, __HIP_MEMORY_SCOPE_AGENT);
        if (__hip_atomic_load((gu32*)err, __ATOMIC_RELAXED, __HIP_MEMORY_SCOPE_AGENT) != 0u) i = 0xffffffffu, lim = 0;
        else if (i >= lim) {
            for (unsigned d = 1; d < 8 && i >= lim; d++) {
                k = (k + 1) & 7u;
                if constexpr (HET) lim = xjobs[k];
                i = __hip_atomic_fetch_add(tickets + 32 * k, 1u, __ATOMIC_RELAXED, __HIP_MEMORY_SCOPE_AGENT);
            }
        }
        if constexpr (HET) {
            const unsigned e = i < lim ? xjobs[8u + k * (unsigned)nstrips + i] : 0xffffffffu;
            job[0] = e != 0xffffffffu ? (int)(e >> 8) : -1;
            job[1] = (int)(e & 255u);
        } else {
            job[0] = i < share ? (int)((i / (unsigned)nstrips) * 8u + k) : -1;
            job[1] = (int)(i % (unsigned)nstrips);
        }
        job[2] = job[3] = 0;
    }
    __syncthreads();
    const int pair = job[0], strip = job[1];
    if (pair < 0 || pair >= n) return;
    size_t fpitch = (size_t)W;
    gu64* cbase;
    if constexpr (HET) {
        const nsof_het_item& it = items[pair];
        W = it.wk;
        H = it.hk;
        if (strip * SW >= W) return;
        R0b += it.offR;
        R1b = R0b + 5 * (size_t)W * H;
        pair_stride = 0;
        flow_in += 2 * it.offF;
        cbase = (gu64*)(carry + it.offR / 2);
        if (het_final) {
            flow_out = it.out;
            fpitch = (size_t)it.out_pitch;
        } else {
            flow_out += 2 * it.offF;
            fpitch = (size_t)W;
        }
    } else {
        if (strip * SW >= W) return;
        cbase = (gu64*)(carry + (size_t)pair * nstrips * (size_t)(((H + 3) / 4) * 40));
    }
    const int nimg = (H + 3) / 4;
    const int x0 = strip * SW;
    const size_t plane = (size_t)W * H;
    const size_t poff = HET ? 0 : (size_t)pair * pair_stride;
    const Planes R0 = planes_of(R0b + poff, plane);
    const Planes R1 = planes_of(R1b + poff, plane);
    const int wave = __builtin_amdgcn_readfirstlane(tid >> 6);
    volatile lds_int* sflag = (volatile lds_int*)(job + 2);
    if (wave < G::NCW) {
        float2* Fout = reinterpret_cast<float2*>(flow_out) + (HET ? 0 : (size_t)pair * plane);
        x_consumer_loop<MH>(ring, sv, vinit, sflag, Fout, fpitch, W, H, x0, tid, nimg, 1. / (block_size * block_size), strip == 0);
    } else if (wave == G::WAVES - 1) {
        float2* Fout = reinterpret_cast<float2*>(flow_out) + (HET ? 0 : (size_t)pair * plane);
        x_solver_loop<MH>(sv, sflag, Fout, fpitch, W, H, x0, nimg, 1. / (block_size * block_size), tid & 63);
    } else if (wave == G::NCW) {
        const int ncols = min(G::SEG0, (W - x0 + 7) & ~7);
        x_scanner_loop<MH>(sv, vinit, cb, strip > 0, nimg, ncols, tid & 63);
    } else {
        const int pw = wave - (G::NCW + 1);
        const int lane = tid & 63;
        FlowSrc F;
        F.base = reinterpret_cast<const char*>(flow_in) + (HET ? 0 : (size_t)pair * plane * 8);
        F.W = (unsigned)W;
        const bool is_io = pw == G::NB;
        const int gp = pw < G::NB ? 0 : 1;
        const int blk = pw < G::NB ? pw : pw - G::NB - 1;
        if (is_io) {
            const int col = G::NB * 64 + (lane & 15), r = lane >> 4;
            const int xc = clampi(x0 - MH - 1 + col, 0, W - 1);
            F.xc = (unsigned)xc;
            const size_t per_strip = (size_t)nimg * 40;
            gu64* cin = strip > 0 ? cbase + (size_t)(strip - 1) * per_strip : nullptr;
            gu64* cout = x0 + SW < W && !((fault & 1) && pair == 0 && strip == 0) ? cbase + (size_t)strip * per_strip : nullptr;
            float2* Fout = reinterpret_cast<float2*>(flow_out) + (HET ? 0 : (size_t)pair * plane);
            x_remainder_loop<MH>(ring, cb, R0, R1, F, W, H, xc, col, r, nimg, cin, cout, epoch, (gu32*)err, sv, sflag + 1, Fout, fpitch,
                                 x0, 1. / (block_size * block_size));
        } else {
            const int col = blk * 64 + lane;
            const int xc = clampi(x0 - MH - 1 + col, 0, W - 1);
            F.xc = (unsigned)xc;
            if (gp == 0)
                x_producer_loop<MH, 0>(ring, R0, R1, F, W, H, xc, col, nimg);
            else
                x_producer_loop<MH, 1>(ring, R0, R1, F, W, H, xc, col, nimg);
        }
    }
}

template <int MH, bool HET>
int launch_x(nsof_ctx* ctx, int n, int max_w, int max_h, const float* R0, const float* R1, size_t pair_stride,
             const float* flow_in, float* flow_out, int W, int H, int winsize, const nsof_het_item* items, bool final,
             const unsigned* xjobs, int stride, int njobs)
{
    using G = XGeom<MH>;
    static_assert(G::SW == NSOF_X_STRIP, "the host's job tables count strips of NSOF_X_STRIP columns");
    if (int rc = lds_opt_in(ctx, k_iterate_x<MH, HET>, G::SMEM)) return rc;
    const int nstrips = HET ? stride : (max_w + G::SW - 1) / G::SW;
    unsigned long long* carry = nullptr;
    unsigned* tickets = nullptr;
    unsigned* err = nullptr;
    const size_t cbytes = HET ? 0 : (size_t)n * nstrips * (size_t)((max_h + 3) / 4) * 40 * 8;
    if (int rc = nsof_xsync_reserve(ctx, cbytes, &carry, &tickets, &err)) return rc;
    NSOF_HIP(ctx, hipMemsetAsync(tickets, 0, 8 * 32 * sizeof(unsigned), ctx->stream));
    unsigned epoch = ++ctx->x_epoch;
    if (epoch == 0) {
        NSOF_HIP(ctx, hipMemsetAsync(ctx->x_carry.p, 0, ctx->x_carry.cap, ctx->stream));
        epoch = ++ctx->x_epoch;
    }
    const unsigned grid = HET ? (unsigned)njobs : 8u * (unsigned)((n + 7) / 8) * (unsigned)nstrips;
    hipLaunchKernelGGL((k_iterate_x<MH, HET>), dim3(grid), dim3(G::THREADS), G::SMEM, ctx->stream, R0, R1, pair_stride, flow_in,
                       flow_out, W, H, winsize, items, final ? 1 : 0, n, nstrips, carry, tickets, epoch, err, ctx->dbg_fault,
                       xjobs);
    return NSOF_OK;
}

}

int nsof_launch_iterate_x(nsof_ctx* ctx, int n_pairs, const float* R0, const float* R1, size_t pair_stride,
                          const float* flow_in, float* flow_out, int W, int H, int winsize)
{
    nsof_prof_scope ps(ctx, NSOF_K_ITERATE);
    int rc = NSOF_OK;
    const bool known = nsof_with_int<1, 7>(winsize / 2, [&](auto mh) {
        rc = launch_x<decltype(mh)::value, false>(ctx, n_pairs, W, H, R0, R1, pair_stride, flow_in, flow_out, W, H, winsize, nullptr,
                                                  false, nullptr, 0, 0);
    });
    if (!known) return nsof_set_error(ctx, NSOF_EUNSUPPORTED, "exact-order fused iteration supports winsize 2..15");
    if (rc) return rc;
    NSOF_HIP(ctx, hipGetLastError());
    return NSOF_OK;
}

int nsof_launch_iterate_x_het(nsof_ctx* ctx, int n_items, const nsof_het_item* d_items, int max_w, int max_h, const float* R,
                              size_t R_floats, const float* flow_in, float* flow_out, bool final, int winsize,
                              const unsigned* d_xjobs, int stride, int njobs)
{
    if (njobs <= 0) return NSOF_OK;
    nsof_prof_scope ps(ctx, NSOF_K_ITERATE);
    unsigned long long* carry;
    unsigned *tk, *er;
    if (int rc0 = nsof_xsync_reserve(ctx, R_floats * 4, &carry, &tk, &er)) return rc0;
    int rc = NSOF_OK;
    const bool known = nsof_with_int<1, 7>(winsize / 2, [&](auto mh) {
        rc = launch_x<decltype(mh)::value, true>(ctx, n_items, max_w, max_h, R, R, (size_t)0, flow_in, flow_out, 0, 0, winsize, d_items,
                                                 final, d_xjobs, stride, njobs);
    });
    if (!known) return nsof_set_error(ctx, NSOF_EUNSUPPORTED, "exact-order fused iteration supports winsize 2..15");
    if (rc) return rc;
    NSOF_HIP(ctx, hipGetLastError());
    return NSOF_OK;
}
```

### neuromorphic-spatiotemporal-optical-flow_amd/csrc/farneback_pyramid.hip

```cpp
#include <cstdlib>

#include <type_traits>

#include "nsof_internal.h"

namespace {

__device__ __forceinline__ void lin_coord_x(int d, double scale, int slen, int& s, float& a)
{
    float f = (float)((d + 0.5) * scale - 0.5);
    s = floor_f(f);
    a = f - s;
    if (s < 0) { s = 0; a = 0.f; }
    if (s >= slen - 1) { s = slen - 1; a = 0.f; }
}
__device__ __forceinline__ void lin_coord_y(int d, double scale, int& s, float& a)
{
    float f = (float)((d + 0.5) * scale - 0.5);
    s = floor_f(f);
    a = f - s;
}


template <typename T>
__device__ __forceinline__ float px(const T* p) { return (float)*p; }
template <typename T>
__device__ __forceinline__ const T* srow(const T* img, ptrdiff_t r, ptrdiff_t stride)
{
    return reinterpret_cast<const T*>(reinterpret_cast<const char*>(img) + r * stride);
}
template <typename T>
constexpr bool kU8 = std::is_same<T, uint8_t>::value;
template <typename T>
constexpr bool kInt = std::is_integral<T>::value;
template <typename T>
constexpr int kPPD = kInt<T> ? 4 / (int)sizeof(T) : 1;
template <typename T>
__device__ __forceinline__ float px_el(unsigned v, int e)
{
    if constexpr (sizeof(T) == 1) return (float)((v >> (8 * e)) & 0xffu);
    else if constexpr (std::is_signed<T>::value) return (float)(int)(short)(v >> (16 * e));
    else return (float)((v >> (16 * e)) & 0xffffu);
}
template <typename T>
using PxQuad = std::conditional_t<sizeof(T) == 2, uint2, float4>;
template <typename T>
__device__ __forceinline__ float quad_el(const PxQuad<T>& v, int e)
{
    if constexpr (sizeof(T) == 2) return px_el<T>(e < 2 ? v.x : v.y, e & 1);
    else return e == 0 ? v.x : (e == 1 ? v.y : (e == 2 ? v.z : v.w));
}

template <int KS, bool FMA, typename TapF, typename LoadF>
__device__ __forceinline__ float row_filter(TapF tk, int ksize, int c, LoadF ld)
{
    const int ks = KS ? KS : ksize, r = ks >> 1;
    if (ks == 3) return nsof_madd<FMA>(ld(c - 1) + ld(c + 1), tk(2), ld(c) * tk(1));
    if (ks == 5) return nsof_madd<FMA>(ld(c - 2) + ld(c + 2), tk(4), nsof_madd<FMA>(ld(c - 1) + ld(c + 1), tk(3), ld(c) * tk(2)));
    float s = tk(0) * ld(c - r);
#pragma unroll
    for (int j = 1; j < ks; j++) s = nsof_madd<FMA>(tk(j), ld(c - r + j), s);
    return s;
}
template <int KS, bool FMA, typename TapF, typename LoadF>
__device__ __forceinline__ float col_filter(TapF tk, int ksize, int rr, LoadF hv)
{
    const int ks = KS ? KS : ksize, r = ks >> 1;
    if (ks == 3) return nsof_madd<FMA>(hv(rr - 1) + hv(rr + 1), tk(2), hv(rr) * tk(1));
    float s = tk(r) * hv(rr);
#pragma unroll
    for (int j = 1; j <= r; j++) s = nsof_madd<FMA>(tk(r + j), hv(rr + j) + hv(rr - j), s);
    return s;
}

template <typename T>
struct PrepImg {
    const T* img;
    float* dst;
};
template <bool HET, typename T>
__device__ __forceinline__ bool prep_geom(PrepImg<T>& g, const T* src, ptrdiff_t& row_stride, ptrdiff_t img_stride,
                                          int& W, int& H, int& wk, int& hk, float* out,
                                          const nsof_het_item* __restrict__ items, int want_flag)
{
    if constexpr (HET) {
        const nsof_het_item& it = items[blockIdx.z >> 1];
        const int which = blockIdx.z & 1;
        if (want_flag >= 0 && (it.flags & NSOF_HET_VEC0) != want_flag) return false;
        W = it.W; H = it.H; wk = it.wk; hk = it.hk;
        row_stride = (ptrdiff_t)it.src_stride[which];
        g.img = reinterpret_cast<const T*>(it.src[which]);
        g.dst = out + it.offI + (size_t)which * wk * hk;
    } else {
        g.img = srow(src, blockIdx.z, img_stride);
        g.dst = out + (size_t)blockIdx.z * wk * hk;
    }
    return true;
}

template <bool HET, typename T, bool FMA>
__global__ __launch_bounds__(256) void k_prep_same(const T* __restrict__ src, ptrdiff_t row_stride,
                                                    ptrdiff_t img_stride, int W, int H, nsof_blur_taps t,
                                                    float* __restrict__ out, const nsof_het_item* __restrict__ items,
                                                    int want_flag)
{
    __shared__ float s_tk[NSOF_MAX_BLUR_TAPS];
    if (threadIdx.x < NSOF_MAX_BLUR_TAPS) s_tk[threadIdx.x] = t.k[threadIdx.x];
    __syncthreads();
    auto tk = [&](int j) { return s_tk[j]; };
    PrepImg<T> g;
    int wk = W, hk = H;
    if (!prep_geom<HET>(g, src, row_stride, img_stride, W, H, wk, hk, out, items, want_flag)) return;
    const int x = blockIdx.x * 64 + (threadIdx.x & 63);
    const int y = blockIdx.y * 4 + (threadIdx.x >> 6);
    if (x >= W || y >= H) return;
    const T* img = g.img;
    auto hv = [&](int rr) {
        const T* rowp = srow(img, reflect101(rr, H), row_stride);
        return row_filter<0, FMA>(tk, t.ksize, x, [&](int c) { return px(rowp + reflect101(c, W)); });
    };
    g.dst[(size_t)y * W + x] = col_filter<0, FMA>(tk, t.ksize, y, hv);
}

constexpr int PREP0_ROWS = 8;
template <bool HET, typename T, bool FMA>
__global__ __launch_bounds__(256) void k_prep_same3_vec(const T* __restrict__ src, ptrdiff_t row_stride,
                                                         ptrdiff_t img_stride, int W, int H, float k0, float k1,
                                                         float* __restrict__ out,
                                                         const nsof_het_item* __restrict__ items)
{
    PrepImg<T> g;
    int wk = W, hk = H;
    if (!prep_geom<HET>(g, src, row_stride, img_stride, W, H, wk, hk, out, items, NSOF_HET_VEC0)) return;
    const int lane = threadIdx.x & 63, wave = threadIdx.x >> 6;
    const int x = (blockIdx.x * 64 + lane) * 4;
    const int y0 = (blockIdx.y * 4 + wave) * PREP0_ROWS;
    if (y0 >= H || blockIdx.x * 256 >= W) return;
    const bool live = x < W;
    const int xl = live ? x : 0;
    const T* img = g.img;
    float* dst = g.dst;

    auto hrow = [&](int rr, float (&h)[4]) {
        const T* rowp = srow(img, reflect101(rr, H), row_stride);
        float s0, s1, s2, s3, sl, sr;
        if constexpr (kU8<T>) {
            const unsigned v = *reinterpret_cast<const unsigned*>(rowp + xl);
            unsigned lft = __shfl_up(v, 1) >> 24, rgt = __shfl_down(v, 1) & 0xffu;
            if (lane == 0 || x == 0) lft = rowp[reflect101(xl - 1, W)];
            if (lane == 63 || x + 4 >= W) rgt = rowp[reflect101(xl + 4, W)];
            s0 = (float)(v & 0xffu); s1 = (float)((v >> 8) & 0xffu); s2 = (float)((v >> 16) & 0xffu);
            s3 = (float)(v >> 24); sl = (float)lft; sr = (float)rgt;
        } else {
            const PxQuad<T> v = *reinterpret_cast<const PxQuad<T>*>(rowp + xl);
            s0 = quad_el<T>(v, 0); s1 = quad_el<T>(v, 1); s2 = quad_el<T>(v, 2); s3 = quad_el<T>(v, 3);
            sl = __shfl_up(s3, 1);
            sr = __shfl_down(s0, 1);
            if (lane == 0 || x == 0) sl = px(rowp + reflect101(xl - 1, W));
            if (lane == 63 || x + 4 >= W) sr = px(rowp + reflect101(xl + 4, W));
        }
        h[0] = nsof_madd<FMA>(sl + s1, k1, s0 * k0);
        h[1] = nsof_madd<FMA>(s0 + s2, k1, s1 * k0);
        h[2] = nsof_madd<FMA>(s1 + s3, k1, s2 * k0);
        h[3] = nsof_madd<FMA>(s2 + sr, k1, s3 * k0);
    };
    float hm[4], h0[4], hp[4];
    hrow(y0 - 1, hm);
    hrow(y0, h0);
#pragma unroll
    for (int q = 0; q < PREP0_ROWS; q++) {
        const int y = y0 + q;
        if (y >= H) break;
        hrow(y + 1, hp);
        if (live) {
            float4 o;
            o.x = nsof_madd<FMA>(hm[0] + hp[0], k1, h0[0] * k0);
            o.y = nsof_madd<FMA>(hm[1] + hp[1], k1, h0[1] * k0);
            o.z = nsof_madd<FMA>(hm[2] + hp[2], k1, h0[2] * k0);
            o.w = nsof_madd<FMA>(hm[3] + hp[3], k1, h0[3] * k0);
            nsof_store_stream4(dst + (size_t)y * W + x, o.x, o.y, o.z, o.w);
        }
#pragma unroll
        for (int i = 0; i < 4; i++) { hm[i] = h0[i]; h0[i] = hp[i]; }
    }
}

template <int S, int KS, int CW, typename T, bool FMA>
__device__ __forceinline__ void prep_decim_body(const T* __restrict__ src, ptrdiff_t row_stride, ptrdiff_t img_stride,
                                                int W, int H, int wk, int hk, int seg_rows, const nsof_blur_taps& t,
                                                float* __restrict__ out, int bx, int seg, int z)
{
    constexpr int R = KS / 2, NPX = CW / S, NC = 2 * NPX;
    constexpr int RING = (KS + 1 + S - 1) / S * S, U = RING / S;
    constexpr int HB = (R + 3) / 4 * 4, HD = HB / 4;
    constexpr int WIN = HB + CW + HB;
    static_assert(NPX >= 1, "lane narrower than one output pixel");
    const int lane = threadIdx.x & 63;
    const int TG = bx * 64 + lane;
    const int dy0 = seg * seg_rows;
    if (dy0 >= hk) return;
    const int dy1 = min(dy0 + seg_rows, hk);
    const bool live = CW * TG < W;
    const int xc0 = live ? CW * TG : 0;
    const bool edge_l = xc0 == 0, edge_r = xc0 + CW >= W;
    const T* img = srow(src, z, img_stride);
    float* dst = out + (size_t)z * wk * hk;
    auto tk = [&](int j) { return t.k[j]; };

    float ring[RING][NC];

    struct RawU8 {
        unsigned cw[CW / 4], hl[HD], hr[HD];
    };
    struct RawQ {
        PxQuad<T> cw[CW / 4], hl[HD], hr[HD];
    };
    using Raw = std::conditional_t<kU8<T>, RawU8, RawQ>;
    auto halo_l = [&](const T* rowp, int d) -> const T* {
        if constexpr (HB > CW) return xc0 - HB + 4 * d >= 0 ? rowp - HB + 4 * d : rowp;
        else return (edge_l ? rowp : rowp - HB) + 4 * d;
    };
    auto halo_r = [&](const T* rowp, int d) -> const T* {
        if constexpr (HB > CW) return xc0 + CW + 4 * d + 4 <= W ? rowp + CW + 4 * d : rowp;
        else return (edge_r ? rowp + (kU8<T> ? 0 : CW - HB) : rowp + CW) + 4 * d;
    };
    auto fetch = [&](int r, Raw& q) {
        const T* rowp = srow(img, reflect101(r, H), row_stride) + xc0;
        if constexpr (!kU8<T>) {
            using Q = PxQuad<T>;
#pragma unroll
            for (int d = 0; d < CW / 4; d++) q.cw[d] = reinterpret_cast<const Q*>(rowp)[d];
#pragma unroll
            for (int d = 0; d < HD; d++) {
                q.hl[d] = *reinterpret_cast<const Q*>(halo_l(rowp, d));
                q.hr[d] = *reinterpret_cast<const Q*>(halo_r(rowp, d));
            }
        } else {
            if (CW == 16) {
                const uint4 c = *reinterpret_cast<const uint4*>(rowp);
                q.cw[0] = c.x; q.cw[1] = c.y; q.cw[(CW / 4 > 2) ? 2 : 0] = c.z; q.cw[(CW / 4 > 3) ? 3 : 0] = c.w;
            } else {
                const uint2 c = *reinterpret_cast<const uint2*>(rowp);
                q.cw[0] = c.x; q.cw[1] = c.y;
            }
#pragma unroll
            for (int d = 0; d < HD; d++) {
                q.hl[d] = *reinterpret_cast<const unsigned*>(halo_l(rowp, d));
                q.hr[d] = *reinterpret_cast<const unsigned*>(halo_r(rowp, d));
            }
        }
    };
    auto filt = [&](const Raw& q, float (&dstrow)[NC]) {
        float raw[WIN];
        if constexpr (kU8<T>) {
#pragma unroll
            for (int b = 0; b < HB; b++) {
                raw[b] = (float)((q.hl[b >> 2] >> (8 * (b & 3))) & 0xffu);
                raw[HB + CW + b] = (float)((q.hr[b >> 2] >> (8 * (b & 3))) & 0xffu);
            }
#pragma unroll
            for (int b = 0; b < CW; b++) raw[HB + b] = (float)((q.cw[b >> 2] >> (8 * (b & 3))) & 0xffu);
        } else {
#pragma unroll
            for (int b = 0; b < HB; b++) {
                raw[b] = quad_el<T>(q.hl[b >> 2], b & 3);
                raw[HB + CW + b] = quad_el<T>(q.hr[b >> 2], b & 3);
            }
#pragma unroll
            for (int b = 0; b < CW; b++) raw[HB + b] = quad_el<T>(q.cw[b >> 2], b & 3);
        }
        float fb[WIN];
#pragma unroll
        for (int b = 0; b < CW; b++) fb[HB + b] = raw[HB + b];
#pragma unroll
        for (int b = 0; b < HB; b++) {
            fb[b] = edge_l ? raw[HB + (HB - b)] : raw[b];
            fb[HB + CW + b] = edge_r ? raw[HB + CW - 2 - b] : raw[HB + CW + b];
        }
#pragma unroll
        for (int n = 0; n < NC; n++) {
            const int off = HB + S * (n >> 1) + S / 2 - 1 + (n & 1);
            dstrow[n] = row_filter<KS, FMA>(tk, KS, off, [&](int q2) { return fb[q2]; });
        }
    };
    auto load_row = [&](int r, float (&dstrow)[NC]) {
        Raw q;
        fetch(r, q);
        filt(q, dstrow);
    };
    constexpr bool PF = S <= (sizeof(T) <= 2 ? 4 : 2);

    const int base = S * dy0 + S / 2 - 1 - R;
#pragma unroll
    for (int i = 0; i <= KS - S; i++) load_row(base + i, ring[i % RING]);

    Raw nx[PF ? S : 1];
    if constexpr (PF) {
#pragma unroll
        for (int i = 0; i < S; i++) fetch(base + KS - S + 1 + i, nx[i]);
    }
    for (int g = 0; dy0 + g * U < dy1; g++) {
#pragma unroll
        for (int u = 0; u < U; u++) {
            const int dy = dy0 + g * U + u;
            if (dy >= dy1) break;
            if constexpr (PF) {
                Raw cu[S];
#pragma unroll
                for (int i = 0; i < S; i++) cu[i] = nx[i];
#pragma unroll
                for (int i = 0; i < S; i++) fetch(base + S * (g * U + u + 1) + KS - S + 1 + i, nx[i]);
#pragma unroll
                for (int i = 0; i < S; i++) filt(cu[i], ring[(S * u + KS - S + 1 + i) % RING]);
            } else {
#pragma unroll
                for (int i = 0; i < S; i++) {
                    load_row(base + S * (g * U + u) + KS - S + 1 + i, ring[(S * u + KS - S + 1 + i) % RING]);
                }
            }
            if (live) {
                float o[NPX];
#pragma unroll
                for (int j = 0; j < NPX; j++) {
                    auto col = [&](int n, int centre) {
// ... 976 lines not shown
```

### neuromorphic-spatiotemporal-optical-flow_amd/csrc/iterate_common.h

```cpp
#pragma once
#include <atomic>
#include <cstdlib>
#include <type_traits>

#include "nsof_internal.h"

namespace {

struct Planes {
    const char* q4;
    const char* c4;
};
struct __attribute__((packed, aligned(4))) f2u {
    float a, b;
};
__device__ __forceinline__ Planes planes_of(const float* img_base, size_t plane)
{
    Planes p;
    p.q4 = reinterpret_cast<const char*>(img_base);
    p.c4 = reinterpret_cast<const char*>(img_base + 4 * plane);
    return p;
}

struct RowIn {
    float4 z;
    float z4;
    float4 t0, t1, b0, b1;
    f2u t4, b4;
    float fx, fy;
    int inside;
};

__device__ __forceinline__ void issue_row(RowIn& in, const Planes& R0, const Planes& R1, int W, int H, int x, int y,
                                          float2 d)
{
    const unsigned pix = (unsigned)y * (unsigned)W + (unsigned)x;
    const float fx = x + d.x, fy = y + d.y;
    const float flx = __builtin_floorf(fx), fly = __builtin_floorf(fy);
    const float xhi = (float)(W - 2), yhi = (float)(H - 2);
    in.fx = fx - flx;
    in.fy = fy - fly;
    in.inside = flx >= 0.f && flx <= xhi && fly >= 0.f && fly <= yhi;
    in.z = *reinterpret_cast<const float4*>(R0.q4 + pix * 16u);
    in.z4 = *reinterpret_cast<const float*>(R0.c4 + pix * 4u);
    const int xs = (int)__builtin_amdgcn_fmed3f(flx, 0.f, xhi), ys = (int)__builtin_amdgcn_fmed3f(fly, 0.f, yhi);
    const unsigned o = (unsigned)ys * (unsigned)W + (unsigned)xs;
    in.t0 = *reinterpret_cast<const float4*>(R1.q4 + o * 16u);
    in.t1 = *reinterpret_cast<const float4*>(R1.q4 + o * 16u + 16u);
    in.b0 = *reinterpret_cast<const float4*>(R1.q4 + (o + (unsigned)W) * 16u);
    in.b1 = *reinterpret_cast<const float4*>(R1.q4 + (o + (unsigned)W) * 16u + 16u);
    in.t4 = *reinterpret_cast<const f2u*>(R1.c4 + o * 4u);
    in.b4 = *reinterpret_cast<const f2u*>(R1.c4 + (o + (unsigned)W) * 4u);
}

__device__ __forceinline__ void matrix_from(const RowIn& in, float dx, float dy, int x, int y, int W, int H, float (&M)[5])
{
    float r2, r3, r4, r5, r6;
    if (in.inside) {
        const float fx = in.fx, fy = in.fy;
        const float a00 = (1.f - fx) * (1.f - fy), a01 = fx * (1.f - fy), a10 = (1.f - fx) * fy, a11 = fx * fy;
        r2 = a00 * in.t0.x + a01 * in.t1.x + a10 * in.b0.x + a11 * in.b1.x;
        r3 = a00 * in.t0.y + a01 * in.t1.y + a10 * in.b0.y + a11 * in.b1.y;
        r4 = a00 * in.t0.z + a01 * in.t1.z + a10 * in.b0.z + a11 * in.b1.z;
        r5 = a00 * in.t0.w + a01 * in.t1.w + a10 * in.b0.w + a11 * in.b1.w;
        r6 = a00 * in.t4.a + a01 * in.t4.b + a10 * in.b4.a + a11 * in.b4.b;
        r4 = (in.z.z + r4) * 0.5f;
        r5 = (in.z.w + r5) * 0.5f;
        r6 = (in.z4 + r6) * 0.25f;
    } else {
        r2 = r3 = 0.f;
        r4 = in.z.z;
        r5 = in.z.w;
        r6 = in.z4 * 0.5f;
    }
    r2 = (in.z.x - r2) * 0.5f;
    r3 = (in.z.y - r3) * 0.5f;
    r2 += r4 * dy + r6 * dx;
    r3 += r6 * dy + r5 * dx;
    if ((unsigned)(x - 5) >= (unsigned)(W - 10) || (unsigned)(y - 5) >= (unsigned)(H - 10)) {
        auto bw = [](int i) { return i < 2 ? 0.14f : 0.4472f; };
        const float scale = (x < 5 ? bw(x) : 1.f) * (x >= W - 5 ? bw(W - x - 1) : 1.f) * (y < 5 ? bw(y) : 1.f) *
                            (y >= H - 5 ? bw(H - y - 1) : 1.f);
        r2 *= scale; r3 *= scale; r4 *= scale; r5 *= scale; r6 *= scale;
    }
    M[0] = r4 * r4 + r6 * r6;
    M[1] = (r4 + r5) * r6;
    M[2] = r5 * r5 + r6 * r6;
    M[3] = r4 * r2 + r6 * r3;
    M[4] = r6 * r2 + r5 * r3;
}

struct FlowSrc {
    const char* base;
    unsigned W, xc;
    __device__ __forceinline__ float2 fetch(int r) const
    {
        return *reinterpret_cast<const float2*>(base + ((unsigned)r * W + xc) * 8u);
    }
};

template <typename K>
int lds_opt_in(nsof_ctx* ctx, K kernel, size_t bytes)
{
    static std::atomic<unsigned long long> done{0};
    const unsigned long long bit = 1ull << (ctx->device & 63);
    if (done.load(std::memory_order_acquire) & bit) return NSOF_OK;
    NSOF_HIP(ctx, hipFuncSetAttribute(reinterpret_cast<const void*>(kernel),
                                      hipFuncAttributeMaxDynamicSharedMemorySize, (int)bytes));
    done.fetch_or(bit, std::memory_order_release);
    return NSOF_OK;
}

}
```

### neuromorphic-spatiotemporal-optical-flow_amd/csrc/nsof_api.hip

```cpp
#include <cctype>
#include <cfloat>
#include <cmath>
#include <cstdlib>
#include <algorithm>
#include <cstring>

#include <sys/syscall.h>
#include <unistd.h>

#include "nsof_internal.h"

static char g_create_err[512] = "";

int nsof_set_error(nsof_ctx* ctx, int code, const char* fmt, ...)
{
    char* dst = ctx ? ctx->err : g_create_err;
    va_list ap;
    va_start(ap, fmt);
    vsnprintf(dst, 512, fmt, ap);
    va_end(ap);
    return code;
}

int nsof_xsync_reserve(nsof_ctx* ctx, size_t carry_bytes, unsigned long long** carry, unsigned** tickets, unsigned** err)
// ... 273 lines not shown
    if (option == NSOF_OPT_ROW_BANDS) {
        *value = ctx->opt_row_bands;
        return NSOF_OK;
    }
    if (option == NSOF_OPT_PYR_FMA) {
        *value = ctx->opt_pyr_fma;
        return NSOF_OK;
    }
    if (option == NSOF_OPT_SMALL_BATCH_JOBS) {
        *value = ctx->opt_small_batch_jobs;
        return NSOF_OK;
    }
    if (option == NSOF_OPT_DEBUG_FAULT) {
        *value = ctx->dbg_fault;
        return NSOF_OK;
    }
    return NSOF_EINVAL;
}

extern "C" int nsof_synchronize(nsof_ctx* ctx)
{
    if (!ctx) return NSOF_EINVAL;
    return nsof_stream_sync_checked(ctx);
}

static int round_half_even(double v) { return (int)lrint(v); }

int nsof_host_blur_taps(int ksize, double sigma, nsof_blur_taps* out)
{
    if (ksize < 1 || (ksize & 1) == 0 || ksize > NSOF_MAX_BLUR_TAPS - 1) return NSOF_EUNSUPPORTED;
    out->ksize = ksize;
    memset(out->k, 0, sizeof(out->k));
    if (sigma <= 0 && ksize <= 9) {
        static const double t1[] = {1.};
        static const double t3[] = {0.25, 0.5, 0.25};
        static const double t5[] = {0.0625, 0.25, 0.375, 0.25, 0.0625};
        static const double t7[] = {0.03125, 0.109375, 0.21875, 0.28125, 0.21875, 0.109375, 0.03125};
        static const double t9[] = {4. / 256, 13. / 256, 30. / 256, 51. / 256, 60. / 256, 51. / 256, 30. / 256, 13. / 256, 4. / 256};
        const double* t = ksize == 1 ? t1 : ksize == 3 ? t3 : ksize == 5 ? t5 : ksize == 7 ? t7 : t9;
        for (int i = 0; i < ksize; i++) out->k[i] = (float)t[i];
        return NSOF_OK;
    }
    const double sg = sigma > 0 ? sigma : ((ksize - 1) * 0.5 - 1) * 0.3 + 0.8;
    const double scale2 = -0.125 / (sg * sg);
    const int h = (ksize - 1) / 2;
    double v[NSOF_MAX_BLUR_TAPS], sum = 0;
    for (int i = 0, x = 1 - ksize; i < h; i++, x += 2) {
        v[i] = std::exp((double)(x * x) * scale2);
        sum += v[i];
    }
    sum = sum * 2.0 + 1.0;
    const double inv = 1.0 / sum;
    for (int i = 0; i < h; i++) out->k[i] = out->k[ksize - 1 - i] = (float)(v[i] * inv);
    out->k[h] = (float)inv;
    return NSOF_OK;
}

static bool chol_inv6(const double A[6][6], double inv[6][6])
{
    double L[6][6] = {{0}};
    for (int i = 0; i < 6; i++)
        for (int j = 0; j <= i; j++) {
            double s = A[i][j];
            for (int k = 0; k < j; k++) s -= L[i][k] * L[j][k];
            if (i == j) {
                if (s <= 0) return false;
                L[i][i] = std::sqrt(s);
            } else
                L[i][j] = s / L[j][j];
        }
    for (int c = 0; c < 6; c++) {
        double y[6], x[6];
        for (int i = 0; i < 6; i++) {
            double s = (i == c) ? 1. : 0.;
            for (int k = 0; k < i; k++) s -= L[i][k] * y[k];
            y[i] = s / L[i][i];
        }
        for (int i = 5; i >= 0; i--) {
            double s = y[i];
            for (int k = i + 1; k < 6; k++) s -= L[k][i] * x[k];
            x[i] = s / L[i][i];
        }
        for (int i = 0; i < 6; i++) inv[i][c] = x[i];
    }
    return true;
}

int nsof_host_poly_taps(int n, double sigma, nsof_poly_taps* out)
{
    if (n < 1 || n > NSOF_MAX_POLY_N) return NSOF_EUNSUPPORTED;
    if (sigma < FLT_EPSILON) sigma = n * 0.3;
    float g[2 * NSOF_MAX_POLY_N + 1], xg[2 * NSOF_MAX_POLY_N + 1], xxg[2 * NSOF_MAX_POLY_N + 1];
    double s = 0.;
    for (int x = -n; x <= n; x++) {
        g[x + n] = (float)std::exp(-x * x / (2 * sigma * sigma));
        s += g[x + n];
    }
    s = 1. / s;
    for (int x = -n; x <= n; x++) {
        g[x + n] = (float)(g[x + n] * s);
        xg[x + n] = (float)(x * g[x + n]);
        xxg[x + n] = (float)(x * x * g[x + n]);
    }
    double G[6][6] = {{0}}, inv[6][6];
    for (int y = -n; y <= n; y++)
        for (int x = -n; x <= n; x++) {
            G[0][0] += g[y + n] * g[x + n];
            G[1][1] += g[y + n] * g[x + n] * x * x;
            G[3][3] += g[y + n] * g[x + n] * x * x * x * x;
            G[5][5] += g[y + n] * g[x + n] * x * x * y * y;
        }
    G[2][2] = G[0][3] = G[0][4] = G[3][0] = G[4][0] = G[1][1];
    G[4][4] = G[3][3];
    G[3][4] = G[4][3] = G[5][5];
    if (!chol_inv6(G, inv)) return NSOF_EINVAL;
    memset(out, 0, sizeof(*out));
    out->n = n;
    for (int k = 0; k <= n; k++) {
        out->g[k] = g[n + k];
        out->xg[k] = xg[n + k];
        out->xxg[k] = xxg[n + k];
        out->dg[k] = (double)g[n + k];
        out->dxxg[k] = (double)xxg[n + k];
    }
    out->ig11 = inv[1][1];
    out->ig03 = inv[0][3];
    out->ig33 = inv[3][3];
    out->ig55 = inv[5][5];
    return NSOF_OK;
}

extern "C" int nsof_farneback_effective_levels(int width, int height, double pyr_scale, int levels)
{
    int k;
    double scale = 1;
    for (k = 0; k < levels; k++) {
        scale *= pyr_scale;
        if (width * scale < 32 || height * scale < 32) break;
    }
    return k;
}

extern "C" int nsof_farneback_level_size(int width, int height, double pyr_scale, int level, int* lw, int* lh,
                                          int* ksize, double* sigma)
{
    if (width < 1 || height < 1 || level < 0 || !(pyr_scale > 0) || !(pyr_scale < 1)) return NSOF_EINVAL;
    double scale = 1;
    for (int i = 0; i < level; i++) scale *= pyr_scale;
    const double sg = (1. / scale - 1) * 0.5;
    int sz = round_half_even(sg * 5) | 1;
    if (sz < 3) sz = 3;
    if (lw) *lw = round_half_even(width * scale);
    if (lh) *lh = round_half_even(height * scale);
    if (ksize) *ksize = sz;
    if (sigma) *sigma = sg;
    return NSOF_OK;
}

int nsof_check_farneback_params(nsof_ctx* ctx, int width, int height, const nsof_fb_params& p)
{
    const int levels = p.levels, winsize = p.winsize, iterations = p.iterations, poly_n = p.poly_n, flags = p.flags;
    if (width < 1 || height < 1) return nsof_set_error(ctx, NSOF_ESHAPE, "empty image %dx%d", width, height);
    if ((long long)width * height > (1ll << 27))
        return nsof_set_error(ctx, NSOF_EUNSUPPORTED, "image %dx%d exceeds 2^27 pixels", width, height);
    if (!(p.pyr_scale > 0) || !(p.pyr_scale < 1))
        return nsof_set_error(ctx, NSOF_EINVAL, "pyr_scale=%g must be in (0,1)", p.pyr_scale);
    if (winsize == 1)
        return nsof_set_error(ctx, NSOF_EUNSUPPORTED, "winsize=1 is not supported");
    if (levels < 0 || winsize < 1 || iterations < 0)
        return nsof_set_error(ctx, NSOF_EINVAL, "levels=%d winsize=%d iterations=%d invalid", levels, winsize,
                              iterations);
    if (poly_n < 1 || poly_n > NSOF_MAX_POLY_N)
        return nsof_set_error(ctx, poly_n < 1 ? NSOF_EINVAL : NSOF_EUNSUPPORTED, "poly_n=%d outside 1..%d", poly_n,
                              NSOF_MAX_POLY_N);
    if (flags != 0 && flags != NSOF_FARNEBACK_GAUSSIAN)
        return nsof_set_error(ctx, NSOF_EUNSUPPORTED,
                              "flags=%d: OPTFLOW_USE_INITIAL_FLOW (4) is not implemented, and no bit other than 256 is known",
                              flags);
    if (flags && winsize / 2 > NSOF_GAUSS_MAX_M)
        return nsof_set_error(ctx, NSOF_EUNSUPPORTED, "winsize=%d too large for the Gaussian window (max %d)", winsize,
                              2 * NSOF_GAUSS_MAX_M + 1);
    return NSOF_OK;
}

int nsof_check_frame_layout(nsof_ctx* ctx, int src, const void* p, ptrdiff_t row_stride, ptrdiff_t img_stride, int width,
                            const char* who, ...)
{
    const ptrdiff_t px = nsof_src_bytes(src);
    if (px == 1 || (reinterpret_cast<uintptr_t>(p) % px == 0 && row_stride % px == 0 && img_stride % px == 0 &&
                    row_stride >= px * width))
        return NSOF_OK;
    char name[64];
    va_list ap;
    va_start(ap, who);
    vsnprintf(name, sizeof(name), who, ap);
    va_end(ap);
    return nsof_set_error(ctx, NSOF_EINVAL, "%s: %td-byte pixels need the address, the row stride (%td) and the image stride (%td) "
                          "to be multiples of %td and the row stride >= %td*width", name, px, row_stride, img_stride, px, px);
}

extern "C" int nsof_stage_pyr_level_px(nsof_ctx* ctx, int pixel_type, int n_img, const void* d_src, ptrdiff_t row_stride,
                                       ptrdiff_t img_stride, int width, int height, double pyr_scale, int level, float* d_out)
{
    if (int rc = nsof_check_typed(ctx, pixel_type)) return rc;
    if (!d_src || !d_out || n_img < 1) return NSOF_EINVAL;
    if (int rc = nsof_check_frame_layout(ctx, pixel_type, d_src, row_stride, img_stride, width, "d_src")) return rc;
    int wk, hk;
    nsof_blur_taps taps;
    if (int rc = nsof_level_geom(ctx, width, height, pyr_scale, level, &wk, &hk, &taps)) return rc;
    return nsof_launch_prep(ctx, n_img, d_src, row_stride, img_stride, width, height, wk, hk, taps, d_out, pixel_type);
}

extern "C" int nsof_stage_pyr_level(nsof_ctx* ctx, int n_img, const uint8_t* d_src, ptrdiff_t row_stride,
                                    ptrdiff_t img_stride, int width, int height, double pyr_scale, int level,
                                    float* d_out)
{
    return nsof_stage_pyr_level_px(ctx, NSOF_PIXEL_U8, n_img, d_src, row_stride, img_stride, width, height, pyr_scale, level, d_out);
}

extern "C" int nsof_stage_pyr_level_f32(nsof_ctx* ctx, int n_img, const float* d_src, ptrdiff_t row_stride,
                                        ptrdiff_t img_stride, int width, int height, double pyr_scale, int level,
                                        float* d_out)
{
    return nsof_stage_pyr_level_px(ctx, NSOF_PIXEL_F32, n_img, d_src, row_stride, img_stride, width, height, pyr_scale, level, d_out);
}

__global__ void k_recip_probe(long long n, const double* __restrict__ x, double* __restrict__ fast, double* __restrict__ ieee)
{
    const long long i = (long long)blockIdx.x * blockDim.x + threadIdx.x;
    if (i < n) {
        fast[i] = nsof_recip_normal(x[i]);
        ieee[i] = 1. / x[i];
    }
}

extern "C" int nsof_stage_recip(nsof_ctx* ctx, long long n, const double* d_x, double* d_out, double* d_ieee)
{
    if (!ctx || !d_x || !d_out || !d_ieee || n < 1) return NSOF_EINVAL;
    hipLaunchKernelGGL(k_recip_probe, dim3((unsigned)((n + 255) / 256)), dim3(256), 0, ctx->stream, n, d_x, d_out, d_ieee);
    NSOF_HIP(ctx, hipGetLastError());
    return NSOF_OK;
}

extern "C" int nsof_stage_polyexp(nsof_ctx* ctx, int n_img, const float* d_img, int width, int height, int poly_n,
                                  double poly_sigma, float* d_R)
{
    if (!ctx || !d_img || !d_R || n_img < 1 || width < 1 || height < 1) return NSOF_EINVAL;
    nsof_poly_taps taps;
    int rc = nsof_host_poly_taps(poly_n, poly_sigma, &taps);
    if (rc) return nsof_set_error(ctx, rc, "poly_n=%d unsupported", poly_n);
    return nsof_launch_polyexp(ctx, n_img, d_img, width, height, taps, d_R);
}

extern "C" int nsof_stage_update_matrices(nsof_ctx* ctx, int n_pairs, const float* d_R, const float* d_flow,
                                          int width, int height, float* d_M)
{
    if (!ctx || !d_R || !d_flow || !d_M || n_pairs < 1 || width < 1 || height < 1) return NSOF_EINVAL;
    const size_t plane = (size_t)width * height;
    return nsof_launch_update_matrices(ctx, n_pairs, d_R, d_R + 5 * plane, 10 * plane, d_flow, width, height, d_M);
}

extern "C" int nsof_stage_blur_solve(nsof_ctx* ctx, int n_pairs, const float* d_M, int width, int height,
                                     int winsize, float* d_flow)
{
    if (!ctx || !d_M || !d_flow || n_pairs < 1 || width < 1 || height < 1 || winsize < 2) return NSOF_EINVAL;
    if (nsof_form_exact(nsof_iterate_form(ctx, winsize, width, height, 1, n_pairs * nsof_iterate_jobs(width, height), 0))) {
        const size_t need = (size_t)n_pairs * 5 * width * height * sizeof(double);
        if (int rc = ctx->ws.reserve(ctx, need)) return rc;
        return nsof_launch_blur_solve_exact(ctx, n_pairs, d_M, width, height, winsize, (double*)ctx->ws.p, d_flow);
    }
    return nsof_launch_blur_solve(ctx, n_pairs, d_M, width, height, winsize, d_flow);
}

extern "C" int nsof_stage_gauss_blur_solve(nsof_ctx* ctx, int n_pairs, const float* d_M, int width, int height,
                                           int winsize, float* d_flow)
{
    if (!ctx || !d_M || !d_flow || n_pairs < 1 || n_pairs > 65535 || width < 1 || height < 1 || winsize < 2) return NSOF_EINVAL;
    return nsof_launch_gauss_blur_solve(ctx, n_pairs, d_M, width, height, winsize, d_flow);
}

extern "C" int nsof_stage_iterate(nsof_ctx* ctx, int n_pairs, const float* d_R, const float* d_flow_in, int width,
                                  int height, int winsize, float* d_flow_out)
{
    if (!ctx || !d_R || !d_flow_in || !d_flow_out || d_flow_in == d_flow_out || n_pairs < 1 || width < 1 || height < 1)
        return NSOF_EINVAL;
    const nsof_iter_form form = nsof_iterate_form(ctx, winsize, width, height, 1, n_pairs * nsof_iterate_jobs(width, height), 0);
    if (!nsof_form_fused(form)) return nsof_set_error(ctx, NSOF_EUNSUPPORTED, "winsize %d not fused", winsize);
    const size_t plane = (size_t)width * height;
    if (form == NSOF_ITER_FAST)
        return nsof_launch_iterate(ctx, n_pairs, d_R, d_R + 5 * plane, 10 * plane, d_flow_in, d_flow_out, width, height,
                                   winsize);
    return nsof_launch_iterate_x(ctx, n_pairs, d_R, d_R + 5 * plane, 10 * plane, d_flow_in, d_flow_out, width, height,
                                 winsize);
}

extern "C" int nsof_stage_iterate_upsample(nsof_ctx* ctx, int n_pairs, const float* d_R, const float* d_coarse_flow,
                                           int src_w, int src_h, int width, int height, int winsize, double pyr_scale,
                                           float* d_flow_out)
{
    if (!ctx || !d_R || !d_coarse_flow || !d_flow_out || n_pairs < 1 || width < 1 || height < 1 || src_w < 1 || src_h < 1)
        return NSOF_EINVAL;
    (void)pyr_scale;
    return nsof_set_error(ctx, NSOF_EUNSUPPORTED, "fused upsample+iteration not available for winsize %d", winsize);
}

extern "C" int nsof_stage_flow_upsample(nsof_ctx* ctx, int n_pairs, const float* d_src, int sw, int sh, float* d_dst,
                                        int dw, int dh, double pyr_scale)
{
    if (!ctx || !d_src || !d_dst || n_pairs < 1 || sw < 1 || sh < 1 || dw < 1 || dh < 1) return NSOF_EINVAL;
    return nsof_launch_flow_upsample(ctx, n_pairs, d_src, sw, sh, d_dst, dw, dh, (float)(1. / pyr_scale));
}

extern "C" int nsof_roi_from_surface(const double* current, int rows, int cols, int frame_w, int frame_h, int memsize,
                                     int thres, int extend_left, int extend_right, int extend_upper, int extend_lower,
                                     int connectivity, int flag, int* rects, int max_rects)
{
    if (!current || rows < 1 || cols < 1 || frame_w < 1 || frame_h < 1 || memsize < 1 || (connectivity != 4 && connectivity != 8) ||
        (flag != 1 && flag != 2) || max_rects < 0 || (max_rects > 0 && !rects))
        return NSOF_EINVAL;
    const int th = frame_h / memsize, tw = frame_w / memsize;
    if (rows > th || cols > tw) return NSOF_ESHAPE;
    std::vector<int> lab((size_t)th * tw, 0);
    std::vector<unsigned char> on((size_t)th * tw, 0);
    for (int y = 0; y < rows; y++)
        for (int x = 0; x < cols; x++) {
            double g = -3366.0 / std::log10(current[(size_t)y * cols + x]) - 306.0;
            g = g < 0.0 ? 0.0 : (g > 255.0 ? 255.0 : g);
            const int gi = (g == g) ? (int)(unsigned char)g : 0;
            on[(size_t)y * tw + x] = gi >= thres;
        }
    struct Box { int x0, y0, x1, y1; };
    std::vector<Box> boxes;
    std::vector<int> stack;
    for (int y = 0; y < th; y++)
        for (int x = 0; x < tw; x++) {
            if (!on[(size_t)y * tw + x] || lab[(size_t)y * tw + x]) continue;
            boxes.push_back({x, y, x, y});
            const int id = (int)boxes.size();
            lab[(size_t)y * tw + x] = id;
            stack.assign(1, y * tw + x);
            while (!stack.empty()) {
                const int p = stack.back();
                stack.pop_back();
                const int py = p / tw, px = p % tw;
                Box& b = boxes[id - 1];
                b.x0 = px < b.x0 ? px : b.x0; b.x1 = px > b.x1 ? px : b.x1;
                b.y0 = py < b.y0 ? py : b.y0; b.y1 = py > b.y1 ? py : b.y1;
                for (int dy = -1; dy <= 1; dy++)
                    for (int dx = -1; dx <= 1; dx++) {
                        if ((!dx && !dy) || (connectivity == 4 && dx && dy)) continue;
                        const int ny = py + dy, nx = px + dx;
                        if (ny < 0 || ny >= th || nx < 0 || nx >= tw) continue;
                        const size_t q = (size_t)ny * tw + nx;
                        if (on[q] && !lab[q]) { lab[q] = id; stack.push_back((int)q); }
                    }
            }
        }
    if (boxes.empty()) return 0;
    if (flag == 2) {
        Box u = boxes[0];
        for (const Box& b : boxes) {
            u.x0 = b.x0 < u.x0 ? b.x0 : u.x0; u.y0 = b.y0 < u.y0 ? b.y0 : u.y0;
            u.x1 = b.x1 > u.x1 ? b.x1 : u.x1; u.y1 = b.y1 > u.y1 ? b.y1 : u.y1;
        }
        boxes.assign(1, u);
    }
    int n = 0;
    for (const Box& b : boxes) {
        const int x0 = std::max(b.x0 * memsize - extend_left, 0), y0 = std::max(b.y0 * memsize - extend_upper, 0);
        const int x1 = std::min((b.x1 + 1) * memsize + extend_right, frame_w), y1 = std::min((b.y1 + 1) * memsize + extend_lower, frame_h);
        if (n < max_rects) { rects[4 * n] = x0; rects[4 * n + 1] = y0; rects[4 * n + 2] = x1; rects[4 * n + 3] = y1; }
        n++;
    }
    return n;
}
```

### neuromorphic-spatiotemporal-optical-flow_amd/csrc/nsof_internal.h

```cpp
#pragma once
#include <hip/hip_runtime.h>

#include <cstdarg>
#include <cstdio>
#include <type_traits>
#include <utility>
#include <vector>

#include "nsof.h"

#define NSOF_MAX_POLY_N 10
#define NSOF_MAX_BLUR_TAPS 64

struct nsof_prof_slot {
    std::vector<hipEvent_t> start, stop;
    size_t used = 0;
    double acc_ms = 0;
    long long acc_launches = 0;
};

struct nsof_ctx;

int nsof_buf_grow(nsof_ctx* ctx, bool pinned, void** p, size_t* cap, size_t need, size_t new_cap);
template <class T, bool Pinned> struct nsof_buf {
    T* p = nullptr;
    size_t cap = 0;
    nsof_buf() = default;
    nsof_buf(const nsof_buf&) = delete;
    nsof_buf& operator=(const nsof_buf&) = delete;
    ~nsof_buf()
    {
        if (p) (void)(Pinned ? hipHostFree((void*)p) : hipFree((void*)p));
    }
    int reserve(nsof_ctx* ctx, size_t need, size_t new_cap) { return nsof_buf_grow(ctx, Pinned, (void**)&p, &cap, need, new_cap); }
    int reserve(nsof_ctx* ctx, size_t need) { return reserve(ctx, need, need); }
    void swap(nsof_buf& o)
    {
        std::swap(p, o.p);
        std::swap(cap, o.cap);
    }
};
template <class T = void> using nsof_dev_buf = nsof_buf<T, false>;
template <class T = void> using nsof_host_buf = nsof_buf<T, true>;

struct nsof_table {
    nsof_host_buf<> h;
    nsof_dev_buf<> d;
    hipEvent_t ev = nullptr;
    ~nsof_table()
    {
        if (ev) (void)hipEventDestroy(ev);
    }
    int stage(nsof_ctx* ctx, size_t bytes, size_t cap);
    const void* upload(nsof_ctx* ctx, size_t bytes);
};

struct nsof_ctx {
    int device = 0;
    hipStream_t stream = nullptr;
    hipStream_t own_stream = nullptr;
    unsigned prof_mask = 0;
    nsof_prof_slot prof[NSOF_K_COUNT];
    int opt_polyexp_f32 = 0;
    int opt_exact_rowsums = 1;
    int opt_row_bands = 0;
    int opt_small_batch_jobs = 64;
    int dbg_fault = 0;
    int opt_pyr_fma = 0;
    char err[512] = {0};
    nsof_dev_buf<> ws;
    nsof_dev_buf<> stage;
    nsof_host_buf<> hstage;
    nsof_dev_buf<> tmp;
    nsof_table het[2];
    int het_flip = 0;
    struct nsof_pipe* pipe = nullptr;
    hipStream_t side = nullptr;
    std::vector<hipEvent_t> ov_events;
    nsof_dev_buf<> roi_tmp;
    nsof_table paste;
    nsof_table seg;
    nsof_table frames;
    nsof_table frame_maps;
    nsof_dev_buf<unsigned long long> x_carry;
    nsof_dev_buf<unsigned> x_sync;
    unsigned x_epoch = 0;
    bool x_dirty = false;
};

int nsof_set_error(nsof_ctx* ctx, int code, const char* fmt, ...);

template <int LO, int HI, class Fn>
bool nsof_with_int(int v, Fn&& f)
{
    if constexpr (LO <= HI) {
        if (v != LO) return nsof_with_int<LO + 1, HI>(v, f);
        f(std::integral_constant<int, LO>{});
        return true;
    } else {
        return false;
    }
}
void* nsof_pinned_alloc(int device, size_t bytes);
int nsof_gpu_numa_node(int device);

#define NSOF_HIP(ctx, call)                                                                      \
    do {                                                                                         \
        hipError_t e_ = (call);                                                                  \
        if (e_ != hipSuccess)                                                                    \
            return nsof_set_error((ctx), NSOF_EDEVICE, "%s failed: %s (%s:%d)", #call,           \
                                  hipGetErrorString(e_), __FILE__, __LINE__);                    \
    } while (0)

struct nsof_prof_scope {
    nsof_ctx* ctx;
    int id;
    bool on;
    nsof_prof_scope(nsof_ctx* c, int k);
    ~nsof_prof_scope();
};

enum nsof_src_type { NSOF_SRC_U8 = 0, NSOF_SRC_F32 = 1, NSOF_SRC_U16 = 2, NSOF_SRC_S16 = 3 };
static inline int nsof_src_bytes(int src) { return src == NSOF_SRC_F32 ? 4 : (src == NSOF_SRC_U8 ? 1 : 2); }
static inline bool nsof_src_valid(int src) { return src >= NSOF_SRC_U8 && src <= NSOF_SRC_S16; }
template <class T> struct nsof_px_tag { using type = T; };
template <class Fn>
bool nsof_with_src_type(int src, Fn&& f)
{
    switch (src) {
        case NSOF_SRC_U8: f(nsof_px_tag<uint8_t>{}); return true;
        case NSOF_SRC_F32: f(nsof_px_tag<float>{}); return true;
        case NSOF_SRC_U16: f(nsof_px_tag<uint16_t>{}); return true;
        case NSOF_SRC_S16: f(nsof_px_tag<int16_t>{}); return true;
        default: return false;
    }
}
static inline int nsof_check_typed(nsof_ctx* ctx, int pixel_type)
{
    if (!ctx) return NSOF_EINVAL;
    return nsof_src_valid(pixel_type) ? NSOF_OK : nsof_set_error(ctx, NSOF_EINVAL, "unknown pixel type %d", pixel_type);
}
int nsof_check_frame_layout(nsof_ctx* ctx, int src, const void* p, ptrdiff_t row_stride, ptrdiff_t img_stride, int width,
                            const char* who, ...) __attribute__((format(printf, 7, 8)));
static inline bool nsof_row_stride_holds(ptrdiff_t row_stride, int width, int src) { return row_stride >= (ptrdiff_t)width * nsof_src_bytes(src); }
static inline size_t align_up(size_t v, size_t a) { return (v + a - 1) / a * a; }
struct nsof_fb_params { double pyr_scale; int levels, winsize, iterations, poly_n; double poly_sigma; int flags; };
int nsof_check_farneback_params(nsof_ctx* ctx, int width, int height, const nsof_fb_params& p);
struct nsof_fb_frames {
    bool sequence;
    int n_pairs;
    const uint8_t *prev, *next;
    ptrdiff_t row_stride, pair_stride;
    int width, height, src;
};
int nsof_farneback_core(nsof_ctx* ctx, const nsof_fb_frames& frames, float* d_flow, const nsof_fb_params& params);
void nsof_pipe_destroy(nsof_ctx* ctx);

struct nsof_blur_taps {
    int ksize;
    float k[NSOF_MAX_BLUR_TAPS];
};
struct nsof_poly_taps {
    int n;
    float g[NSOF_MAX_POLY_N + 1], xg[NSOF_MAX_POLY_N + 1], xxg[NSOF_MAX_POLY_N + 1];
    double dg[NSOF_MAX_POLY_N + 1], dxxg[NSOF_MAX_POLY_N + 1];
    double ig11, ig03, ig33, ig55;
};

int nsof_host_blur_taps(int ksize, double sigma, nsof_blur_taps* out);
static inline int nsof_level_geom(nsof_ctx* ctx, int width, int height, double pyr_scale, int level, int* wk, int* hk,
                                  nsof_blur_taps* bt)
{
    int ks;
    double sg;
    int rc = nsof_farneback_level_size(width, height, pyr_scale, level, wk, hk, &ks, &sg);
    if (rc) return ctx ? nsof_set_error(ctx, rc, "bad level geometry") : rc;
    if ((rc = nsof_host_blur_taps(ks, sg, bt)) && ctx)
        return nsof_set_error(ctx, rc, "pyramid blur kernel size %d unsupported (max %d)", ks, NSOF_MAX_BLUR_TAPS - 1);
    return rc;
}
int nsof_host_poly_taps(int n, double sigma, nsof_poly_taps* out);
static inline bool nsof_level0_from_frames(const nsof_ctx* ctx, int src, const nsof_blur_taps& bt)
{
    return src != NSOF_SRC_F32 && !ctx->opt_pyr_fma && !ctx->opt_polyexp_f32 && bt.ksize == 3;
}

struct nsof_het_item {
    const uint8_t* src[2];
    long long src_stride[2];
    float* out;
    long long out_pitch;
    unsigned long long offI, offR, offF, offFc;
    int W, H;
    int wk, hk;
    int pw, ph;
    int flags;
    int pad_;
};
enum { NSOF_HET_VEC0 = 1 };

int nsof_launch_update_matrices(nsof_ctx* ctx, int n_pairs, const float* R0, const float* R1, size_t pair_stride,
                                const float* flow, int W, int H, float* M);
int nsof_launch_iterate_lat(nsof_ctx* ctx, int n_pairs, const float* R0, const float* R1, size_t pair_stride,
                            const float* flow_in, float* flow_out, int W, int H, int winsize, float* M, double* V);
int nsof_launch_iterate_lat_het(nsof_ctx* ctx, int n_items, const nsof_het_item* d_items, int max_w, int max_h, const float* R,
                                const float* flow_in, float* flow_out, bool final, int winsize, float* M, double* V);
int nsof_launch_prep_het(nsof_ctx* ctx, int n_items, const nsof_het_item* d_items, const nsof_het_item* h_items,
                         bool level0, const nsof_blur_taps& taps, float* I, int src_type);
int nsof_launch_polyexp_het(nsof_ctx* ctx, int n_items, const nsof_het_item* d_items, int max_w, int max_h,
                            const nsof_poly_taps& taps, const float* I, float* R, const float* blur3,
                            int src_type);
int nsof_launch_flow_upsample_het(nsof_ctx* ctx, int n_items, const nsof_het_item* d_items, int max_w, int max_h,
                                  const float* src, float* dst, float mul);
int nsof_launch_iterate_het(nsof_ctx* ctx, int n_items, const nsof_het_item* d_items, int max_w, const float* R,
                            const float* flow_in, float* flow_out, bool final, int winsize);
int nsof_launch_prep(nsof_ctx* ctx, int n_img, const void* src, ptrdiff_t row_stride, ptrdiff_t img_stride, int W,
                     int H, int wk, int hk, const nsof_blur_taps& taps, float* out, int src_type);
int nsof_launch_prep_decim3(nsof_ctx* ctx, int n_img, const void* src, ptrdiff_t row_stride, ptrdiff_t img_stride, int W,
                            int H, const nsof_blur_taps* taps, float* const* out, int src_type);
int nsof_launch_polyexp(nsof_ctx* ctx, int n_img, const float* img, int W, int H, const nsof_poly_taps& taps,
                        float* R);
int nsof_launch_polyexp_frames(nsof_ctx* ctx, int n_img, const void* src0, const void* src1, int nsplit, ptrdiff_t row_stride,
                           ptrdiff_t img_stride, int W, int H, const nsof_poly_taps& taps, float k0, float k1, float* R,
                           int src_type);
int nsof_launch_blur_solve(nsof_ctx* ctx, int n_pairs, const float* M, int W, int H, int winsize, float* flow);
int nsof_launch_blur_solve_exact(nsof_ctx* ctx, int n_pairs, const float* M, int W, int H, int winsize, double* VT,
                                 float* flow);
#define NSOF_GAUSS_LDS_MAX_M 16
#define NSOF_GAUSS_MAX_M 96
struct nsof_gauss_taps {
    float k[NSOF_GAUSS_MAX_M + 1];
};
int nsof_launch_gauss_blur_solve(nsof_ctx* ctx, int n_pairs, const float* M, int W, int H, int winsize, float* flow);
int nsof_launch_flow_upsample(nsof_ctx* ctx, int n_pairs, const float* src, int sw, int sh, float* dst, int dw,
                              int dh, float mul);
int nsof_launch_iterate(nsof_ctx* ctx, int n_pairs, const float* R0, const float* R1, size_t pair_stride,
                        const float* flow_in, float* flow_out, int W, int H, int winsize);
int nsof_launch_iterate_x(nsof_ctx* ctx, int n_pairs, const float* R0, const float* R1, size_t pair_stride,
                          const float* flow_in, float* flow_out, int W, int H, int winsize);
#define NSOF_X_STRIP 192
int nsof_launch_iterate_x_het(nsof_ctx* ctx, int n_items, const nsof_het_item* d_items, int max_w, int max_h, const float* R,
                              size_t R_floats, const float* flow_in, float* flow_out, bool final, int winsize,
                              const unsigned* d_xjobs, int stride, int njobs);

static inline bool nsof_iterate_supported(int winsize, int W, int H)
{
    const int m = winsize / 2;
    return m >= 1 && m <= 7 && W >= 2 && H >= 2;
}
static inline long long nsof_iterate_jobs(int W, int H)
{
    return (unsigned long long)W * H * 40ull < (1ull << 32) ? (W + NSOF_X_STRIP - 1) / NSOF_X_STRIP : 1ll << 31;
}
enum nsof_iter_form {
    NSOF_ITER_FAST,
    NSOF_ITER_EXACT,
    NSOF_ITER_EXACT_LAT,
    NSOF_ITER_UNFUSED_FAST,
    NSOF_ITER_UNFUSED_EXACT,
    NSOF_ITER_UNFUSED_GAUSS,
};
static inline nsof_iter_form nsof_iterate_form(const nsof_ctx* ctx, int winsize, int W, int H, int iterations, long long jobs,
                                               int flags)
{
    if (flags & NSOF_FARNEBACK_GAUSSIAN) return NSOF_ITER_UNFUSED_GAUSS;
    const bool fused = nsof_iterate_supported(winsize, W, H);
    if (!ctx->opt_exact_rowsums) return fused ? NSOF_ITER_FAST : NSOF_ITER_UNFUSED_FAST;
    if (!fused || iterations < 1) return NSOF_ITER_UNFUSED_EXACT;
    return jobs <= ctx->opt_small_batch_jobs ? NSOF_ITER_EXACT_LAT : NSOF_ITER_EXACT;
}
static inline bool nsof_form_fused(nsof_iter_form f) { return f <= NSOF_ITER_EXACT_LAT; }
static inline bool nsof_form_exact(nsof_iter_form f) { return f != NSOF_ITER_FAST && f != NSOF_ITER_UNFUSED_FAST; }
int nsof_xsync_reserve(nsof_ctx* ctx, size_t carry_bytes, unsigned long long** carry, unsigned** tickets, unsigned** err);
int nsof_xsync_check(nsof_ctx* ctx);
int nsof_stream_sync_checked(nsof_ctx* ctx);

#ifdef __HIPCC__
typedef float nsof_f4v __attribute__((ext_vector_type(4)));
typedef float nsof_f2v __attribute__((ext_vector_type(2)));
__device__ __forceinline__ double nsof_recip_normal(double x)
{
    double r = __builtin_amdgcn_rcp(x);
    double e = __builtin_fma(-x, r, 1.0);
    r = __builtin_fma(r, e, r);
    e = __builtin_fma(-x, r, 1.0);
    r = __builtin_fma(r, e, r);
    e = __builtin_fma(-x, r, 1.0);
    return __builtin_fma(e, r, r);
}

__device__ __forceinline__ float2 nsof_flow_solve(double s0, double s1, double s2, double s3, double s4, double scale)
{
    const double g11 = s0 * scale, g12 = s1 * scale, g22 = s2 * scale, h1 = s3 * scale, h2 = s4 * scale;
    const double idet = nsof_recip_normal(g11 * g22 - g12 * g12 + 1e-3);
    return make_float2((float)((g11 * h2 - g12 * h1) * idet), (float)((g22 * h1 - g12 * h2) * idet));
}

__device__ __forceinline__ int clampi(int v, int lo, int hi) { return v < lo ? lo : (v > hi ? hi : v); }
__device__ __forceinline__ int reflect101(int p, int len)
{
    if ((unsigned)p < (unsigned)len) return p;
    if (len == 1) return 0;
    do {
        if (p < 0) p = -p;
        else p = 2 * len - 2 - p;
    } while ((unsigned)p >= (unsigned)len);
    return p;
}
template <bool FMA>
__device__ __forceinline__ float nsof_madd(float a, float b, float c)
{
    if constexpr (FMA) return fmaf(a, b, c);
    else return a * b + c;
}
__device__ __forceinline__ int floor_f(float v)
{
    if (!(v >= -2147483648.0f && v < 2147483648.0f)) return v < 0.f ? 2147483647 : -2147483647 - 1;
    int i = (int)v;
    return i - (i > v);
}

__device__ __forceinline__ unsigned nsof_gray_px(unsigned c0, unsigned c1, unsigned c2, int w0, int w1, int w2)
{
    return (c0 * w0 + c1 * w1 + c2 * w2 + (1u << 14)) >> 15;
}

__device__ __forceinline__ void nsof_store_stream4(float* p, float a, float b, float c, float d)
{
    __builtin_nontemporal_store((nsof_f4v){a, b, c, d}, reinterpret_cast<nsof_f4v*>(p));
}
__device__ __forceinline__ void nsof_store_stream2(float* p, float a, float b)
{
    __builtin_nontemporal_store((nsof_f2v){a, b}, reinterpret_cast<nsof_f2v*>(p));
}
#endif
```

### neuromorphic-spatiotemporal-optical-flow_amd/nsof/_lib.py

```python
import ctypes as C
import importlib.util
import os


_HERE = os.path.dirname(os.path.abspath(__file__))
LIB_PATH = os.environ.get("NSOF_LIB", os.path.join(_HERE, "libnsof.so"))

OPT_POLYEXP_F32 = 1
OPT_EXACT_ROWSUMS = 2
OPT_ROW_BANDS = 3
OPT_PYR_FMA = 4
OPT_SMALL_BATCH_JOBS = 5
OPT_DEBUG_FAULT = 100
NSOF_OK, NSOF_EINVAL, NSOF_ESHAPE, NSOF_EDEVICE, NSOF_ENOMEM, NSOF_EUNSUPPORTED = 0, -1, -2, -3, -4, -5
PIXEL_U8, PIXEL_F32, PIXEL_U16, PIXEL_S16 = 0, 1, 2, 3
ACCUM_KEYS = ("alphaoff", "alphaon", "voff", "von", "koff", "kon", "son", "soff", "bon", "boff", "Ron", "Roff", "wini")
K_PREP, K_POLYEXP, K_UPSAMPLE, K_UPDMAT, K_BLUR, K_ACCUM, K_ITERATE, K_SEGMENT, K_MORPH, K_REMAP, K_SSIM, K_COUNT = range(12)

_vp, _i, _d, _f, _sz, _pd, _i64 = C.c_void_p, C.c_int, C.c_double, C.c_float, C.c_size_t, C.c_ssize_t, C.c_int64

class PairDesc(C.Structure):
    _fields_ = [("prev", _vp), ("prev_stride", _pd), ("next", _vp), ("next_stride", _pd), ("width", _i), ("height", _i),
                ("flow", _vp), ("flow_stride", _pd)]


class AccumParams(C.Structure):
    _fields_ = [(k, _d) for k in ("alphaoff", "alphaon", "voff", "von", "koff", "kon", "son", "soff", "bon", "boff", "Ron",
                                  "Roff", "wini", "dt")] + [("refractory_us", _i64)]


_ap = C.POINTER(AccumParams)
_ll = C.POINTER(C.c_longlong)
_fb = [_d, _i, _i, _i, _i, _d, _i]
_TYPED = {
    "nsof_farneback_px": [_vp, _i, _vp, _pd, _vp, _pd, _i, _i, _vp, _pd] + _fb,
    "nsof_farneback_px_batch_dev": [_vp, _i, _i, _vp, _vp, _pd, _pd, _i, _i, _vp] + _fb,
    "nsof_farneback_px_sequence_dev": [_vp, _i, _i, _vp, _pd, _pd, _i, _i, _vp] + _fb,
    "nsof_farneback_px_batch": [_vp, _i, _i, C.POINTER(PairDesc)] + _fb,
    "nsof_farneback_px_batch_desc_dev": [_vp, _i, _i, C.POINTER(PairDesc)] + _fb,
    "nsof_farneback_px_roi_sequence_dev": [_vp, _i, _i, _vp, _pd, _pd, _i, _i, _vp, _vp, _i, _vp] + _fb + [_i, _ll, _ll],
    "nsof_stage_pyr_level_px": [_vp, _i, _i, _vp, _pd, _pd, _i, _i, _d, _i, _vp],
}


def _typed_signatures():
    out = {}
    for name, args in _TYPED.items():
        out[name] = (_i, args)
        for infix in ("" if name.startswith("nsof_stage") else "_u8", "_f32"):
            out[name.replace("_px", infix, 1)] = (_i, args[:1] + args[2:])
    return out


SIGNATURES = {
    **_typed_signatures(),
    "nsof_create": (_i, [_i, C.POINTER(_vp)]),
    "nsof_destroy": (None, [_vp]),
    "nsof_last_error": (C.c_char_p, [_vp]),
    "nsof_abi_version": (_i, []),
    "nsof_set_stream": (_i, [_vp, _vp]),
    "nsof_synchronize": (_i, [_vp]),
    "nsof_set_option": (_i, [_vp, _i, _i]),
    "nsof_get_option": (_i, [_vp, _i, C.POINTER(_i)]),
    "nsof_host_alloc": (_vp, [_sz]),
    "nsof_host_free": (None, [_vp]),
    "nsof_farneback_effective_levels": (_i, [_i, _i, _d, _i]),
    "nsof_farneback_level_size": (_i, [_i, _i, _d, _i, C.POINTER(_i), C.POINTER(_i), C.POINTER(_i), C.POINTER(_d)]),
    "nsof_stage_polyexp": (_i, [_vp, _i, _vp, _i, _i, _i, _d, _vp]),
    "nsof_stage_recip": (_i, [_vp, C.c_longlong, _vp, _vp, _vp]),
    "nsof_stage_update_matrices": (_i, [_vp, _i, _vp, _vp, _i, _i, _vp]),
    "nsof_stage_blur_solve": (_i, [_vp, _i, _vp, _i, _i, _i, _vp]),
    "nsof_stage_gauss_blur_solve": (_i, [_vp, _i, _vp, _i, _i, _i, _vp]),
    "nsof_stage_iterate": (_i, [_vp, _i, _vp, _vp, _i, _i, _i, _vp]),
    "nsof_stage_iterate_upsample": (_i, [_vp, _i, _vp, _vp, _i, _i, _i, _i, _i, _d, _vp]),
    "nsof_stage_flow_upsample": (_i, [_vp, _i, _vp, _i, _i, _vp, _i, _i, _d]),
    "nsof_prof_enable": (_i, [_vp, C.c_uint]),
    "nsof_prof_collect": (_i, [_vp, _i, C.POINTER(_d), C.POINTER(C.c_longlong)]),
    "nsof_kernel_name": (C.c_char_p, [_i]),
    "nsof_accum_create": (_i, [_vp, _i, _i, _i, _i, _f, _f, C.POINTER(_vp)]),
    "nsof_accum_default_params": (None, [_ap]),
    "nsof_accum_create_p": (_i, [_vp, _i, _i, _i, _i, _f, _f, _ap, C.POINTER(_vp)]),
    "nsof_accum_get_params": (_i, [_vp, _ap]),
    "nsof_accum_update_state_p_dev": (_i, [_vp, _ap, _vp, _vp, _vp, _sz]),
    "nsof_accum_resistance_p_dev": (_i, [_vp, _ap, _vp, _vp, _sz]),
    "nsof_accum_frames_f64_p": (_i, [_vp, _vp, _i, _i, _i, _d, _i, _d, _d, _ap, _vp, _vp]),
    "nsof_accum_frames_f64_p_dev": (_i, [_vp, _vp, _i, _i, _i, _d, _i, _d, _d, _d, _ap, _vp, _vp, _vp]),
    "nsof_accum_frames_f64_maps_dev": (_i, [_vp, _vp, _i, _i, _i, _d, _i, _d, _d, _d, _ap, _i, _i, C.POINTER(_i), C.POINTER(_vp),
                                            C.POINTER(_i), _vp, _vp, _vp]),
    "nsof_accum_frames_f64_maps": (_i, [_vp, _vp, _i, _i, _i, _d, _i, _d, _d, _ap, _i, _i, C.POINTER(_i), C.POINTER(_vp),
                                        C.POINTER(_i), _vp, _vp]),
    "nsof_accum_trials_dev": (_i, [_vp, _i, _i, _i, _i, _f, _f, _ap, _i, _vp, _vp, _vp, _vp, _vp, _i64, _i64, _i, _d, _i, _i,
                                   C.POINTER(_i), C.POINTER(_vp), C.POINTER(_i), _vp, _vp, _vp]),
    "nsof_gate_stats_dev": (_i, [_vp, _vp, _vp, _i, _i, _i, _i, _i, _vp, _vp]),
    "nsof_accum_destroy": (None, [_vp]),
    "nsof_accum_set_param_maps": (_i, [_vp, _i, C.POINTER(_i), C.POINTER(_vp)]),
    "nsof_accum_read_param_map": (_i, [_vp, _i, _vp]),
    "nsof_accum_param_map_mask": (_i, [_vp, C.POINTER(C.c_uint)]),
    "nsof_accum_set_dense": (_i, [_vp, _i]),
    "nsof_accum_set_event_threshold": (_i, [_vp, _i]),
    "nsof_accum_get_event_threshold": (_i, [_vp, _vp]),
    "nsof_accum_reset": (_i, [_vp]),
    "nsof_accum_step_events": (_i, [_vp, _vp, _vp, _vp, _vp, _vp, _i64, _i64]),
    "nsof_accum_set_events": (_i, [_vp, _vp, _vp, _vp, _vp, _vp, _i64]),
    "nsof_accum_set_slice_times": (_i, [_vp, _vp, _vp, _i64]),
    "nsof_accum_run": (_i, [_vp, _i64, _i64, _i64]),
    "nsof_accum_surface_u8_dev": (_i, [_vp, _i, _i, _vp, _pd]),
    "nsof_accum_surface_f32_dev": (_i, [_vp, _i, _i, _vp, _pd]),
    "nsof_accum_run_surface": (_i, [_vp, _i64, _i64, _i, _i, _vp, _pd]),
    "nsof_accum_run_frames": (_i, [_vp, _i64, _i64, _i64, _i, _i, _vp, _pd, _pd]),
    "nsof_accum_set_frames_path": (_i, [_vp, _i]),
    "nsof_accum_read_state": (_i, [_vp, _i, _vp, _vp, C.POINTER(_i64)]),
    "nsof_accum_write_state": (_i, [_vp, _i, _vp, _vp, _i64]),
    "nsof_accum_update_state_dev": (_i, [_vp, _vp, _vp, _vp, _sz]),
    "nsof_accum_resistance_dev": (_i, [_vp, _vp, _vp, _sz]),
    "nsof_accum_bincount_2d": (_i, [_vp, _vp, _vp, _sz, _i, _i, _vp]),
    "nsof_accum_read_w": (_i, [_vp, _i, _vp]),
    "nsof_accum_read_resistance": (_i, [_vp, _i, _vp]),
    "nsof_accum_snapshot_count": (_i64, [_vp]),
    "nsof_accum_read_snapshots": (_i, [_vp, _i, _vp, _i64]),
    "nsof_accum_block_current": (_i, [_vp, _i, _i64, _i, _d, _vp]),
    "nsof_accum_block_current_dev": (_i, [_vp, _i, _i64, _i, _d, _vp]),
    "nsof_accum_frames_f64": (_i, [_vp, _vp, _i, _i, _i, _d, _i, _d, _d, _vp, _vp]),
    "nsof_accum_frames_f64_dev": (_i, [_vp, _vp, _i, _i, _i, _d, _i, _d, _d, _d, _vp, _vp, _vp]),
    "nsof_frames_compress_u8_dev": (_i, [_vp, _i, _vp, _pd, _pd, _i, _i, _i, _i, _vp, _vp, _i, _vp, _vp, _i, _vp]),
    "nsof_lanczos3_contributions": (_i, [_i, _i, _vp, _vp, _i, C.POINTER(_i)]),
    "nsof_accum_slice_bounds": (_i64, [_vp, _i64, _i64, _vp, _i64]),
    "nsof_roi_from_surface": (_i, [_vp, _i, _i, _i, _i, _i, _i, _i, _i, _i, _i, _i, _i, _vp, _i]),
    "nsof_roi_from_surface_dev": (_i, [_vp, _vp, _i, _sz, _i, _i, _i, _i, _i, _i, _i, _i, _i, _i, _i, _i, _i, _vp, _vp, _vp]),
    "nsof_structuring_element": (_i, [_i, _i, _i, _vp]),
    "nsof_morph_binary_u8_dev": (_i, [_vp, _i, _vp, _pd, _i, _i, _vp, _i, _i, _i, _i, _i, _vp, _pd]),
    "nsof_motion_mask_dev": (_i, [_vp, _vp, _pd, _i, _i, _d, _i, _i, _vp, _pd]),
    "nsof_motion_mask": (_i, [_vp, _vp, _pd, _i, _i, _d, _i, _i, _vp, _pd]),
    "nsof_motion_mask_sequence_dev": (_i, [_vp, _i, _vp, _i, _i, _vp, _vp, _d, _i, _i, _vp]),
    "nsof_pixel_accuracy_u8_batch_dev": (_i, [_vp, _i, _vp, _vp, _pd, _pd, _i, _i, _vp]),
    "nsof_gray_u8_dev": (_i, [_vp, _vp, _pd, _i, _i, _i, _vp, _pd]),
    "nsof_remap_linear_u8_dev": (_i, [_vp, _vp, _pd, _i, _i, _i, _vp, _pd, _vp, _pd, _i, _i, _i, _i, _vp, _pd]),
    "nsof_predict_warp_u8_dev": (_i, [_vp, _vp, _pd, _i, _i, _i, _vp, _pd, _i, _i, _i, _i, _i, _i, _vp, _pd]),
    "nsof_predict_warp_u8": (_i, [_vp, _vp, _pd, _i, _i, _i, _vp, _pd, _i, _i, _i, _i, _i, _i, _vp, _pd]),
    "nsof_ssim_u8_dev": (_i, [_vp, _vp, _pd, _i, _vp, _pd, _i, _i, _i, _d, C.POINTER(_d)]),
    "nsof_ssim_u8": (_i, [_vp, _vp, _pd, _i, _vp, _pd, _i, _i, _i, _d, C.POINTER(_d)]),
    "nsof_predict_sequence_u8_dev": (_i, [_vp, _i, _vp, _pd, _pd, _i, _i, _vp, _i, _vp, _vp, _i, _i, _i, _i, _i, _vp]),
    "nsof_ssim_u8_batch_dev": (_i, [_vp, _i, _vp, _pd, _pd, _i, _vp, _pd, _pd, _i, _i, _i, _d, _vp]),
    "nsof_flow_to_image_dev": (_i, [_vp, _i, _vp, _pd, _pd, _i, _i, _i, _d, _d, _i, _vp, _pd, _pd, _vp]),
}

_lib = None


def _preload_torch_hip_runtime():
    if os.environ.get("NSOF_HIP_RUNTIME", "") == "system":
        return
    try:
        spec = importlib.util.find_spec("torch")
    except (ImportError, ValueError):
        spec = None
    if spec is None or not spec.submodule_search_locations:
        return
    cand = os.path.join(list(spec.submodule_search_locations)[0], "lib", "libamdhip64.so")
    if os.path.exists(cand):
        C.CDLL(cand, mode=C.RTLD_GLOBAL)


def load():
    global _lib
    if _lib is None:
        if not os.path.exists(LIB_PATH):
            raise OSError(
                f"{LIB_PATH} not found: build it with `make -C {os.path.dirname(_HERE)}` "
                "(or `python -c 'import __graft_entry__ as g; g.build()'`); nsof has no CPU fallback")
        _preload_torch_hip_runtime()
        lib = C.CDLL(LIB_PATH)
        for name, (res, args) in SIGNATURES.items():
            fn = getattr(lib, name)
            fn.restype = res
            fn.argtypes = args
        _lib = lib
    return _lib
```

Before: 7120.

## Fuse 2x flow upsampling into first exact iteration of each pyramid level

Adds a FlowResample2x flow source and a k_iterate_xr kernel. When the form is the exact fused iteration and the level is exactly twice the coarser size, the first iteration now bilinearly resamples the coarse flow on the fly instead of running a separate upsample kernel. This removes one kernel launch and one full-resolution flow write and read per level. In exchange, each flow sample needs four coarse loads and extra arithmetic inside the producer waves, and the buffer-flip parity is recomputed to match.

After: 7482, median of 6. 5.1% higher.

```diff
diff --git a/include/nsof.h b/include/nsof.h
--- a/include/nsof.h
+++ b/include/nsof.h
@@ -189,6 +189,9 @@
 int nsof_stage_iterate_upsample(nsof_ctx* ctx, int n_pairs, const float* d_R, const float* d_coarse_flow,
                                 int src_w, int src_h, int width, int height, int winsize, double pyr_scale,
                                 float* d_flow_out);
+int nsof_stage_iterate_x_resample(nsof_ctx* ctx, int n_pairs, const float* d_R, const float* d_coarse_flow,
+                                  int src_w, int src_h, int width, int height, int winsize, double pyr_scale,
+                                  float* d_flow_out);
 int nsof_stage_flow_upsample(nsof_ctx* ctx, int n_pairs, const float* d_src, int src_w, int src_h,
                              float* d_dst, int dst_w, int dst_h, double pyr_scale);
 
diff --git a/neuromorphic-spatiotemporal-optical-flow_amd/csrc/farneback_driver.hip b/neuromorphic-spatiotemporal-optical-flow_amd/csrc/farneback_driver.hip
--- a/neuromorphic-spatiotemporal-optical-flow_amd/csrc/farneback_driver.hip
+++ b/neuromorphic-spatiotemporal-optical-flow_amd/csrc/farneback_driver.hip
@@ -118,7 +118,12 @@
     return rc == NSOF_EUNSUPPORTED ? NSOF_OK : rc;
 }
 
-static int iterate_level(const Run& r, int k, int wk, int hk, float* const fb[2], int* cur)
+static bool first_iteration_resamples(const Run& r, int wk, int hk, int pw, int ph)
+{
+    return r.form == NSOF_ITER_EXACT && r.p.iterations >= 1 && wk == 2 * pw && hk == 2 * ph && !r.ctx->opt_pyr_fma;
+}
+
+static int iterate_level(const Run& r, int k, int wk, int hk, float* const fb[2], int* cur, int pw, int ph)
 {
     nsof_ctx* ctx = r.ctx;
     const int n_pairs = r.f.n_pairs, winsize = r.p.winsize;
@@ -133,6 +138,9 @@
             float* in = fb[*cur];
             float* out = fb[*cur ^= 1];
             if (r.form == NSOF_ITER_EXACT_LAT) rc = nsof_launch_iterate_lat(ctx, n_pairs, R0, R1, 5 * nk, in, out, wk, hk, winsize, dM, dV);
+            else if (r.form == NSOF_ITER_EXACT && it == 0 && pw > 0)
+                rc = nsof_launch_iterate_x_resample(ctx, n_pairs, R0, R1, 5 * nk, in, pw, ph, (float)(1. / r.p.pyr_scale), out, wk, hk,
+                                                    winsize);
             else if (r.form == NSOF_ITER_EXACT) rc = nsof_launch_iterate_x(ctx, n_pairs, R0, R1, 5 * nk, in, out, wk, hk, winsize);
             else rc = nsof_launch_iterate(ctx, n_pairs, R0, R1, 5 * nk, in, out, wk, hk, winsize);
         } else {
@@ -157,7 +165,14 @@
     if ((rc = ctx->ws.reserve(ctx, r.cv.total()))) return rc;
     r.cv.base = (char*)ctx->ws.p;
     float* const fb[2] = {d_flow, r.cv.S()};
-    const int flips = nsof_form_fused(r.form) ? L * (1 + iterations) + iterations : L;
+    int flips = nsof_form_fused(r.form) ? L * (1 + iterations) + iterations : L;
+    for (int k = L, cw = 0, ch = 0; k >= 0; k--) {
+        int wk, hk;
+        nsof_farneback_level_size(f.width, f.height, r.p.pyr_scale, k, &wk, &hk, nullptr, nullptr);
+        if (k < L && first_iteration_resamples(r, wk, hk, cw, ch)) flips--;
+        cw = wk;
+        ch = hk;
+    }
     int cur = flips & 1;
 
     const hipStream_t mainS = ctx->stream;
@@ -170,9 +185,10 @@
         int wk, hk;
         nsof_blur_taps btaps;
         if ((rc = nsof_level_geom(ctx, f.width, f.height, r.p.pyr_scale, k, &wk, &hk, &btaps))) return rc;
+        const bool resample_in_first = k < L && first_iteration_resamples(r, wk, hk, pw, ph);
         if (k == L) {
             NSOF_HIP(ctx, hipMemsetAsync(fb[cur], 0, r.B * wk * hk * 8, mainS));
-        } else {
+        } else if (!resample_in_first) {
             if ((rc = nsof_launch_flow_upsample(ctx, f.n_pairs, fb[cur], pw, ph, fb[cur ^ 1], wk, hk, (float)(1. / r.p.pyr_scale))))
                 return rc;
             cur ^= 1;
@@ -182,7 +198,7 @@
         } else if (k < L) {
             NSOF_HIP(ctx, hipStreamWaitEvent(mainS, ctx->ov_events[k], 0));
         }
-        if ((rc = iterate_level(r, k, wk, hk, fb, &cur))) return rc;
+        if ((rc = iterate_level(r, k, wk, hk, fb, &cur, resample_in_first ? pw : 0, ph))) return rc;
         pw = wk;
         ph = hk;
     }
diff --git a/neuromorphic-spatiotemporal-optical-flow_amd/csrc/farneback_iterate_x.hip b/neuromorphic-spatiotemporal-optical-flow_amd/csrc/farneback_iterate_x.hip
--- a/neuromorphic-spatiotemporal-optical-flow_amd/csrc/farneback_iterate_x.hip
+++ b/neuromorphic-spatiotemporal-optical-flow_amd/csrc/farneback_iterate_x.hip
@@ -51,26 +51,32 @@
 
 constexpr unsigned X_SPIN_LIMIT = 1u << 21;
 
-template <int MH>
-__device__ __forceinline__ void x_produce(RowIn& in, float2& dd, float2& fl, const XRing& ring, const Planes& R0,
-                                          const Planes& R1, const FlowSrc& F, int W, int H, int xc, int col, int i)
+template <int MH, class FS>
+__device__ __forceinline__ void x_produce(RowIn& in, float2& dd, typename FS::Pend& fl, const XRing& ring, const Planes& R0,
+                                          const Planes& R1, const FS& F, int W, int H, int xc, int col, int i)
 {
     constexpr int RL = XGeom<MH>::RL;
     float Mn[5];
     matrix_from(in, dd.x, dd.y, xc, min(i, H - 1), W, H, Mn);
     ring.put((i + MH + 1) % RL, col, Mn);
-    issue_row(in, R0, R1, W, H, xc, min(i + 8, H - 1), fl);
-    dd = fl;
+    const int y = min(i + 8, H - 1);
+    dd = F.value(fl, y);
+    issue_row(in, R0, R1, W, H, xc, y, dd);
     fl = F.fetch(min(i + 16, H - 1));
 }
 
-template <int MH>
-__device__ __forceinline__ void x_rows_above(const XRing& ring, const Planes& R0, const Planes& R1, const FlowSrc& F,
+template <int MH, class FS>
+__device__ __forceinline__ void x_rows_above(const XRing& ring, const Planes& R0, const Planes& R1, const FS& F,
                                              int W, int H, int xc, int col)
 {
     float2 fl[MH];
-#pragma unroll
-    for (int i = 0; i < MH; i++) fl[i] = F.fetch(min(i, H - 1));
+    {
+        typename FS::Pend pd[MH];
+#pragma unroll
+        for (int i = 0; i < MH; i++) pd[i] = F.fetch(min(i, H - 1));
+#pragma unroll
+        for (int i = 0; i < MH; i++) fl[i] = F.value(pd[i], min(i, H - 1));
+    }
     constexpr int GRP = 4;
 #pragma unroll
     for (int g0 = 0; g0 < MH; g0 += GRP) {
@@ -93,19 +99,20 @@
     }
 }
 
-template <int MH, int GP>
+template <int MH, int GP, class FS>
 __device__ __forceinline__ void x_producer_loop(const XRing& ring, const Planes& R0, const Planes& R1,
-                                                const FlowSrc& F, int W, int H, int xc, int col, int nimg)
+                                                const FS& F, int W, int H, int xc, int col, int nimg)
 {
     if constexpr (GP == 0) x_rows_above<MH>(ring, R0, R1, F, W, H, xc, col);
     RowIn in[2][2];
-    float2 dd[2][2], fl[2][2];
+    float2 dd[2][2];
+    typename FS::Pend fl[2][2];
 #pragma unroll
     for (int ts = 0; ts < 2; ts++)
 #pragma unroll
         for (int rr = 0; rr < 2; rr++) {
             const int r = min(4 * ts + MH + 2 * GP + rr, H - 1);
-            dd[ts][rr] = F.fetch(r);
+            dd[ts][rr] = F.value(F.fetch(r), r);
             issue_row(in[ts][rr], R0, R1, W, H, xc, r, dd[ts][rr]);
         }
 #pragma unroll
@@ -134,6 +141,66 @@
     }
 }
 
+template <int MH, int GP>
+__device__ __forceinline__ void x_producer_loop(const XRing& ring, const Planes& R0, const Planes& R1,
+                                                const FlowResample2x& F, int W, int H, int xc, int col, int nimg)
+{
+    constexpr int RL = XGeom<MH>::RL;
+    constexpr bool ODD = (MH & 1) != 0;
+    if constexpr (GP == 0) x_rows_above<MH>(ring, R0, R1, F, W, H, xc, col);
+    RowIn in[2][2];
+    float2 dd[2][2];
+    {
+        FlowResample2x::Pend p[2][2];
+#pragma unroll
+        for (int ts = 0; ts < 2; ts++)
+#pragma unroll
+            for (int rr = 0; rr < 2; rr++) p[ts][rr] = F.fetch(min(4 * ts + MH + 2 * GP + rr, H - 1));
+#pragma unroll
+        for (int ts = 0; ts < 2; ts++)
+#pragma unroll
+            for (int rr = 0; rr < 2; rr++) {
+                const int r = min(4 * ts + MH + 2 * GP + rr, H - 1);
+                dd[ts][rr] = F.value(p[ts][rr], r);
+                issue_row(in[ts][rr], R0, R1, W, H, xc, r, dd[ts][rr]);
+            }
+    }
+    float2 z = make_float2(0.f, 0.f);
+    if constexpr (!ODD) z = F.upper_row(min(8 + MH + 2 * GP, H - 1));
+    FlowResample2x::Pend2 pd = F.template fetch2<ODD>(min(8 + MH + 2 * GP, H - 1), min(9 + MH + 2 * GP, H - 1));
+    auto step = [&](auto tsc, int t) {
+        constexpr int TS = decltype(tsc)::value;
+        const int i = 4 * t + MH + 2 * GP;
+#pragma unroll
+        for (int rr = 0; rr < 2; rr++) {
+            float Mn[5];
+            matrix_from(in[TS][rr], dd[TS][rr].x, dd[TS][rr].y, xc, min(i + rr, H - 1), W, H, Mn);
+            ring.put((i + rr + MH + 1) % RL, col, Mn);
+        }
+        const int ya = min(i + 8, H - 1), yb = min(i + 9, H - 1);
+        F.template value2<ODD>(pd, z, ya, yb, dd[TS][0], dd[TS][1]);
+        pd = F.template fetch2<ODD>(min(i + 12, H - 1), min(i + 13, H - 1));
+        asm volatile("" ::: "memory");
+        issue_row(in[TS][0], R0, R1, W, H, xc, ya, dd[TS][0]);
+        issue_row(in[TS][1], R0, R1, W, H, xc, yb, dd[TS][1]);
+    };
+    step(std::integral_constant<int, 0>{}, 0);
+    __syncthreads();
+    step(std::integral_constant<int, 1>{}, 1);
+    __syncthreads();
+    int t = 0;
+    for (; t < nimg; t += 2) {
+        step(std::integral_constant<int, 0>{}, t + 2);
+        __syncthreads();
+        step(std::integral_constant<int, 1>{}, t + 3);
+        __syncthreads();
+    }
+    if (t == nimg) {
+        step(std::integral_constant<int, 0>{}, t + 2);
+        __syncthreads();
+    }
+}
+
 template <int MH, int Q0, int NQ>
 __device__ __forceinline__ void x_solve_rows(const double* sv, volatile lds_int* flag, float2* Fout, size_t fpitch, int W, int H,
                                              int x0, int nimg, double scale, int lane, int t)
@@ -168,9 +235,9 @@
     }
 }
 
-template <int MH>
+template <int MH, class FS>
 __device__ __forceinline__ void x_remainder_loop(const XRing& ring, double* cb, const Planes& R0, const Planes& R1,
-                                                 const FlowSrc& F, int W, int H, int xc, int col, int r, int nimg,
+                                                 const FS& F, int W, int H, int xc, int col, int r, int nimg,
                                                  gu64* cin, gu64* cout, unsigned epoch, gu32* err, const double* sv,
                                                  volatile lds_int* ioflag, float2* Fout, size_t fpitch, int x0, double scale)
 {
@@ -214,11 +281,12 @@
     };
     if (r == 0) x_rows_above<MH>(ring, R0, R1, F, W, H, xc, col);
     RowIn in[2];
-    float2 dd[2], fl[2];
+    float2 dd[2];
+    typename FS::Pend fl[2];
 #pragma unroll
     for (int ts = 0; ts < 2; ts++) {
         const int y = min(4 * ts + MH + r, H - 1);
-        dd[ts] = F.fetch(y);
+        dd[ts] = F.value(F.fetch(y), y);
         issue_row(in[ts], R0, R1, W, H, xc, y, dd[ts]);
     }
 #pragma unroll
@@ -507,12 +575,12 @@
     }
 }
 
-template <int MH, bool HET>
-__global__ __launch_bounds__((XGeom<MH>::THREADS)) void k_iterate_x(
+template <int MH, bool HET, class FS>
+__device__ __forceinline__ void x_walk(
     const float* __restrict__ R0b, const float* __restrict__ R1b, size_t pair_stride, const float* __restrict__ flow_in,
     float* __restrict__ flow_out, int W, int H, int block_size, const nsof_het_item* __restrict__ items, int het_final,
     int n, int nstrips, unsigned long long* carry, unsigned* tickets, unsigned epoch, unsigned* err, int fault,
-    const unsigned* __restrict__ xjobs)
+    const unsigned* __restrict__ xjobs, FS F)
 {
     using G = XGeom<MH>;
     constexpr int SW = G::SW, COLS = G::COLS;
@@ -595,16 +663,14 @@
     } else {
         const int pw = wave - (G::NCW + 1);
         const int lane = tid & 63;
-        FlowSrc F;
-        F.base = reinterpret_cast<const char*>(flow_in) + (HET ? 0 : (size_t)pair * plane * 8);
-        F.W = (unsigned)W;
+        F.template bind<HET>(flow_in, pair, plane, W);
         const bool is_io = pw == G::NB;
         const int gp = pw < G::NB ? 0 : 1;
         const int blk = pw < G::NB ? pw : pw - G::NB - 1;
         if (is_io) {
             const int col = G::NB * 64 + (lane & 15), r = lane >> 4;
             const int xc = clampi(x0 - MH - 1 + col, 0, W - 1);
-            F.xc = (unsigned)xc;
+            F.column(xc);
             const size_t per_strip = (size_t)nimg * 40;
             gu64* cin = strip > 0 ? cbase + (size_t)(strip - 1) * per_strip : nullptr;
             gu64* cout = x0 + SW < W && !((fault & 1) && pair == 0 && strip == 0) ? cbase + (size_t)strip * per_strip : nullptr;
@@ -614,13 +680,50 @@
         } else {
             const int col = blk * 64 + lane;
             const int xc = clampi(x0 - MH - 1 + col, 0, W - 1);
-            F.xc = (unsigned)xc;
+            F.column(xc);
             if (gp == 0)
                 x_producer_loop<MH, 0>(ring, R0, R1, F, W, H, xc, col, nimg);
             else
                 x_producer_loop<MH, 1>(ring, R0, R1, F, W, H, xc, col, nimg);
         }
     }
+}
+
+template <int MH, bool HET>
+__global__ __launch_bounds__((XGeom<MH>::THREADS)) void k_iterate_x(
+    const float* __restrict__ R0b, const float* __restrict__ R1b, size_t pair_stride, const float* __restrict__ flow_in,
+    float* __restrict__ flow_out, int W, int H, int block_size, const nsof_het_item* __restrict__ items, int het_final,
+    int n, int nstrips, unsigned long long* carry, unsigned* tickets, unsigned epoch, unsigned* err, int fault,
+    const unsigned* __restrict__ xjobs)
+{
+    x_walk<MH, HET>(R0b, R1b, pair_stride, flow_in, flow_out, W, H, block_size, items, het_final, n, nstrips, carry, tickets, epoch,
+                    err, fault, xjobs, FlowSrc{});
+}
+
+template <int MH>
+__global__ __launch_bounds__((XGeom<MH>::THREADS)) void k_iterate_xr(
+    const float* __restrict__ R0b, const float* __restrict__ R1b, size_t pair_stride, const float* __restrict__ coarse,
+    int pw, int ph, float mul, float* __restrict__ flow_out, int W, int H, int block_size, int n, int nstrips,
+    unsigned long long* carry, unsigned* tickets, unsigned epoch, unsigned* err, int fault)
+{
+    FlowResample2x F;
+    F.pw = (unsigned)pw;
+    F.ph = ph;
+    F.mul = mul;
+    x_walk<MH, false>(R0b, R1b, pair_stride, coarse, flow_out, W, H, block_size, nullptr, 0, n, nstrips, carry, tickets, epoch, err,
+                      fault, nullptr, F);
+}
+
+int x_launch_state(nsof_ctx* ctx, size_t cbytes, unsigned long long** carry, unsigned** tickets, unsigned** err, unsigned* epoch)
+{
+    if (int rc = nsof_xsync_reserve(ctx, cbytes, carry, tickets, err)) return rc;
+    NSOF_HIP(ctx, hipMemsetAsync(*tickets, 0, 8 * 32 * sizeof(unsigned), ctx->stream));
+    *epoch = ++ctx->x_epoch;
+    if (*epoch == 0) {
+        NSOF_HIP(ctx, hipMemsetAsync(ctx->x_carry.p, 0, ctx->x_carry.cap, ctx->stream));
+        *epoch = ++ctx->x_epoch;
+    }
+    return NSOF_OK;
 }
 
 template <int MH, bool HET>
@@ -635,18 +738,32 @@
     unsigned long long* carry = nullptr;
     unsigned* tickets = nullptr;
     unsigned* err = nullptr;
+    unsigned epoch = 0;
     const size_t cbytes = HET ? 0 : (size_t)n * nstrips * (size_t)((max_h + 3) / 4) * 40 * 8;
-    if (int rc = nsof_xsync_reserve(ctx, cbytes, &carry, &tickets, &err)) return rc;
-    NSOF_HIP(ctx, hipMemsetAsync(tickets, 0, 8 * 32 * sizeof(unsigned), ctx->stream));
-    unsigned epoch = ++ctx->x_epoch;
-    if (epoch == 0) {
-        NSOF_HIP(ctx, hipMemsetAsync(ctx->x_carry.p, 0, ctx->x_carry.cap, ctx->stream));
-        epoch = ++ctx->x_epoch;
-    }
+    if (int rc = x_launch_state(ctx, cbytes, &carry, &tickets, &err, &epoch)) return rc;
     const unsigned grid = HET ? (unsigned)njobs : 8u * (unsigned)((n + 7) / 8) * (unsigned)nstrips;
     hipLaunchKernelGGL((k_iterate_x<MH, HET>), dim3(grid), dim3(G::THREADS), G::SMEM, ctx->stream, R0, R1, pair_stride, flow_in,
                        flow_out, W, H, winsize, items, final ? 1 : 0, n, nstrips, carry, tickets, epoch, err, ctx->dbg_fault,
                        xjobs);
+    return NSOF_OK;
+}
+
+template <int MH>
+int launch_xr(nsof_ctx* ctx, int n, const float* R0, const float* R1, size_t pair_stride, const float* coarse, int pw, int ph,
+              float mul, float* flow_out, int W, int H, int winsize)
+{
+    using G = XGeom<MH>;
+    if (int rc = lds_opt_in(ctx, k_iterate_xr<MH>, G::SMEM)) return rc;
+    const int nstrips = (W + G::SW - 1) / G::SW;
+    unsigned long long* carry = nullptr;
+    unsigned* tickets = nullptr;
+    unsigned* err = nullptr;
+    unsigned epoch = 0;
+    const size_t cbytes = (size_t)n * nstrips * (size_t)((H + 3) / 4) * 40 * 8;
+    if (int rc = x_launch_state(ctx, cbytes, &carry, &tickets, &err, &epoch)) return rc;
+    const unsigned grid = 8u * (unsigned)((n + 7) / 8) * (unsigned)nstrips;
+    hipLaunchKernelGGL((k_iterate_xr<MH>), dim3(grid), dim3(G::THREADS), G::SMEM, ctx->stream, R0, R1, pair_stride, coarse, pw, ph,
+                       mul, flow_out, W, H, winsize, n, nstrips, carry, tickets, epoch, err, ctx->dbg_fault);
     return NSOF_OK;
 }
 
@@ -662,6 +779,23 @@
                                                   false, nullptr, 0, 0);
     });
     if (!known) return nsof_set_error(ctx, NSOF_EUNSUPPORTED, "exact-order fused iteration supports winsize 2..15");
+    if (rc) return rc;
+    NSOF_HIP(ctx, hipGetLastError());
+    return NSOF_OK;
+}
+
+int nsof_launch_iterate_x_resample(nsof_ctx* ctx, int n_pairs, const float* R0, const float* R1, size_t pair_stride,
+                                   const float* coarse_flow, int pw, int ph, float mul, float* flow_out, int W, int H, int winsize)
+{
+    if (pw < 1 || ph < 1 || W != 2 * pw || H != 2 * ph)
+        return nsof_set_error(ctx, NSOF_EUNSUPPORTED, "resampling iteration: %dx%d is not the double of %dx%d", W, H, pw, ph);
+    if (winsize < 2 || winsize > 15)
+        return nsof_set_error(ctx, NSOF_EUNSUPPORTED, "exact-order fused iteration supports winsize 2..15");
+    nsof_prof_scope ps(ctx, NSOF_K_ITERATE);
+    int rc = NSOF_OK;
+    nsof_with_int<1, 7>(winsize / 2, [&](auto mh) {
+        rc = launch_xr<decltype(mh)::value>(ctx, n_pairs, R0, R1, pair_stride, coarse_flow, pw, ph, mul, flow_out, W, H, winsize);
+    });
     if (rc) return rc;
     NSOF_HIP(ctx, hipGetLastError());
     return NSOF_OK;
diff --git a/neuromorphic-spatiotemporal-optical-flow_amd/csrc/farneback_pyramid.hip b/neuromorphic-spatiotemporal-optical-flow_amd/csrc/farneback_pyramid.hip
--- a/neuromorphic-spatiotemporal-optical-flow_amd/csrc/farneback_pyramid.hip
+++ b/neuromorphic-spatiotemporal-optical-flow_amd/csrc/farneback_pyramid.hip
@@ -6,20 +6,6 @@
 
 namespace {
 
-__device__ __forceinline__ void lin_coord_x(int d, double scale, int slen, int& s, float& a)
-{
-    float f = (float)((d + 0.5) * scale - 0.5);
-    s = floor_f(f);
-    a = f - s;
-    if (s < 0) { s = 0; a = 0.f; }
-    if (s >= slen - 1) { s = slen - 1; a = 0.f; }
-}
-__device__ __forceinline__ void lin_coord_y(int d, double scale, int& s, float& a)
-{
-    float f = (float)((d + 0.5) * scale - 0.5);
-    s = floor_f(f);
-    a = f - s;
-}
 
 
 template <typename T>
diff --git a/neuromorphic-spatiotemporal-optical-flow_amd/csrc/iterate_common.h b/neuromorphic-spatiotemporal-optical-flow_amd/csrc/iterate_common.h
--- a/neuromorphic-spatiotemporal-optical-flow_amd/csrc/iterate_common.h
+++ b/neuromorphic-spatiotemporal-optical-flow_amd/csrc/iterate_common.h
@@ -91,11 +91,109 @@
 }
 
 struct FlowSrc {
+    typedef float2 Pend;
     const char* base;
     unsigned W, xc;
+    template <bool HET>
+    __device__ __forceinline__ void bind(const float* field, int pair, size_t plane, int w)
+    {
+        base = reinterpret_cast<const char*>(field) + (HET ? 0 : (size_t)pair * plane * 8);
+        W = (unsigned)w;
+    }
+    __device__ __forceinline__ void column(int c) { xc = (unsigned)c; }
     __device__ __forceinline__ float2 fetch(int r) const
     {
         return *reinterpret_cast<const float2*>(base + ((unsigned)r * W + xc) * 8u);
+    }
+    __device__ __forceinline__ float2 value(const float2& p, int) const { return p; }
+};
+
+struct FlowResample2x {
+    struct Pend {
+        float2 p00, p01, p10, p11;
+    };
+    struct Pend2 {
+        float2 x0, x1, y0, y1;
+    };
+    const char* base;
+    unsigned pw;
+    int ph;
+    float mul;
+    int sy0, sy1;
+    float b10, b11;
+    unsigned c0, c1;
+    float a0, a1;
+    template <bool HET>
+    __device__ __forceinline__ void bind(const float* field, int pair, size_t, int)
+    {
+        static_assert(!HET, "uniform batches only");
+        base = reinterpret_cast<const char*>(field) + (size_t)pair * pw * (size_t)ph * 8;
+        lin_coord_y(0, 0.5, sy0, b10);
+        lin_coord_y(1, 0.5, sy1, b11);
+        sy0 = __builtin_amdgcn_readfirstlane(sy0);
+        sy1 = __builtin_amdgcn_readfirstlane(sy1);
+        b10 = __builtin_bit_cast(float, __builtin_amdgcn_readfirstlane(__builtin_bit_cast(int, b10)));
+        b11 = __builtin_bit_cast(float, __builtin_amdgcn_readfirstlane(__builtin_bit_cast(int, b11)));
+    }
+    __device__ __forceinline__ void column(int c)
+    {
+        int sx;
+        lin_coord_x(c, 0.5, (int)pw, sx, a1);
+        a0 = 1.f - a1;
+        c0 = (unsigned)sx * 8u;
+        c1 = (unsigned)min(sx + 1, (int)pw - 1) * 8u;
+    }
+    __device__ __forceinline__ int row_sy(int r) const { return (r >> 1) + ((r & 1) ? sy1 : sy0); }
+    __device__ __forceinline__ float row_b1(int r) const { return (r & 1) ? b11 : b10; }
+    __device__ __forceinline__ unsigned row_off(int cr) const { return (unsigned)clampi(cr, 0, ph - 1) * pw * 8u; }
+    __device__ __forceinline__ float2 at(unsigned off) const { return *reinterpret_cast<const float2*>(base + off); }
+    __device__ __forceinline__ float2 hblend(const float2& p0, const float2& p1) const
+    {
+        return make_float2(nsof_madd<false>(p0.x, a0, p1.x * a1), nsof_madd<false>(p0.y, a0, p1.y * a1));
+    }
+    __device__ __forceinline__ float2 vblend(const float2& t0, const float2& t1, int r) const
+    {
+        const float b1 = row_b1(r), b0 = 1.f - b1;
+        return make_float2(nsof_madd<false>(t0.x, b0, t1.x * b1) * mul, nsof_madd<false>(t0.y, b0, t1.y * b1) * mul);
+    }
+    __device__ __forceinline__ Pend fetch(int r) const
+    {
+        const int sy = row_sy(r);
+        const unsigned r0 = row_off(sy), r1 = row_off(sy + 1);
+        Pend p;
+        p.p00 = at(r0 + c0);
+        p.p01 = at(r0 + c1);
+        p.p10 = at(r1 + c0);
+        p.p11 = at(r1 + c1);
+        return p;
+    }
+    __device__ __forceinline__ float2 value(const Pend& p, int r) const
+    {
+        return vblend(hblend(p.p00, p.p01), hblend(p.p10, p.p11), r);
+    }
+    template <bool ODD>
+    __device__ __forceinline__ Pend2 fetch2(int ra, int rb) const
+    {
+        const unsigned rx = row_off(row_sy(ra) + (ODD ? 0 : 1)), ry = row_off((ODD ? row_sy(ra) : row_sy(rb)) + 1);
+        Pend2 q;
+        q.x0 = at(rx + c0);
+        q.x1 = at(rx + c1);
+        q.y0 = at(ry + c0);
+        q.y1 = at(ry + c1);
+        return q;
+    }
+    template <bool ODD>
+    __device__ __forceinline__ void value2(const Pend2& q, float2& z, int ra, int rb, float2& oa, float2& ob) const
+    {
+        const float2 hx = hblend(q.x0, q.x1), hy = hblend(q.y0, q.y1);
+        oa = ODD ? vblend(hx, hy, ra) : vblend(z, hx, ra);
+        ob = vblend(hx, hy, rb);
+        z = hy;
+    }
+    __device__ __forceinline__ float2 upper_row(int r) const
+    {
+        const unsigned r0 = row_off(row_sy(r));
+        return hblend(at(r0 + c0), at(r0 + c1));
     }
 };
 
diff --git a/neuromorphic-spatiotemporal-optical-flow_amd/csrc/nsof_api.hip b/neuromorphic-spatiotemporal-optical-flow_amd/csrc/nsof_api.hip
--- a/neuromorphic-spatiotemporal-optical-flow_amd/csrc/nsof_api.hip
+++ b/neuromorphic-spatiotemporal-optical-flow_amd/csrc/nsof_api.hip
@@ -599,6 +599,18 @@
         return NSOF_EINVAL;
     (void)pyr_scale;
     return nsof_set_error(ctx, NSOF_EUNSUPPORTED, "fused upsample+iteration not available for winsize %d", winsize);
+}
+
+extern "C" int nsof_stage_iterate_x_resample(nsof_ctx* ctx, int n_pairs, const float* d_R, const float* d_coarse_flow,
+                                             int src_w, int src_h, int width, int height, int winsize, double pyr_scale,
+                                             float* d_flow_out)
+{
+    if (!ctx || !d_R || !d_coarse_flow || !d_flow_out || d_coarse_flow == d_flow_out || n_pairs < 1 || width < 1 || height < 1 ||
+        src_w < 1 || src_h < 1)
+        return NSOF_EINVAL;
+    const size_t plane = (size_t)width * height;
+    return nsof_launch_iterate_x_resample(ctx, n_pairs, d_R, d_R + 5 * plane, 10 * plane, d_coarse_flow, src_w, src_h,
+                                          (float)(1. / pyr_scale), d_flow_out, width, height, winsize);
 }
 
 extern "C" int nsof_stage_flow_upsample(nsof_ctx* ctx, int n_pairs, const float* d_src, int sw, int sh, float* d_dst,
diff --git a/neuromorphic-spatiotemporal-optical-flow_amd/csrc/nsof_internal.h b/neuromorphic-spatiotemporal-optical-flow_amd/csrc/nsof_internal.h
--- a/neuromorphic-spatiotemporal-optical-flow_amd/csrc/nsof_internal.h
+++ b/neuromorphic-spatiotemporal-optical-flow_amd/csrc/nsof_internal.h
@@ -238,6 +238,9 @@
                         const float* flow_in, float* flow_out, int W, int H, int winsize);
 int nsof_launch_iterate_x(nsof_ctx* ctx, int n_pairs, const float* R0, const float* R1, size_t pair_stride,
                           const float* flow_in, float* flow_out, int W, int H, int winsize);
+int nsof_launch_iterate_x_resample(nsof_ctx* ctx, int n_pairs, const float* R0, const float* R1, size_t pair_stride,
+                                   const float* coarse_flow, int pw, int ph, float mul, float* flow_out, int W, int H,
+                                   int winsize);
 #define NSOF_X_STRIP 192
 int nsof_launch_iterate_x_het(nsof_ctx* ctx, int n_items, const nsof_het_item* d_items, int max_w, int max_h, const float* R,
                               size_t R_floats, const float* flow_in, float* flow_out, bool final, int winsize,
@@ -319,6 +322,20 @@
     int i = (int)v;
     return i - (i > v);
 }
+__device__ __forceinline__ void lin_coord_x(int d, double scale, int slen, int& s, float& a)
+{
+    float f = (float)((d + 0.5) * scale - 0.5);
+    s = floor_f(f);
+    a = f - s;
+    if (s < 0) { s = 0; a = 0.f; }
+    if (s >= slen - 1) { s = slen - 1; a = 0.f; }
+}
+__device__ __forceinline__ void lin_coord_y(int d, double scale, int& s, float& a)
+{
+    float f = (float)((d + 0.5) * scale - 0.5);
+    s = floor_f(f);
+    a = f - s;
+}
 
 __device__ __forceinline__ unsigned nsof_gray_px(unsigned c0, unsigned c1, unsigned c2, int w0, int w1, int w2)
 {
diff --git a/neuromorphic-spatiotemporal-optical-flow_amd/nsof/_lib.py b/neuromorphic-spatiotemporal-optical-flow_amd/nsof/_lib.py
--- a/neuromorphic-spatiotemporal-optical-flow_amd/nsof/_lib.py
+++ b/neuromorphic-spatiotemporal-optical-flow_amd/nsof/_lib.py
@@ -73,6 +73,7 @@
     "nsof_stage_gauss_blur_solve": (_i, [_vp, _i, _vp, _i, _i, _i, _vp]),
     "nsof_stage_iterate": (_i, [_vp, _i, _vp, _vp, _i, _i, _i, _vp]),
     "nsof_stage_iterate_upsample": (_i, [_vp, _i, _vp, _vp, _i, _i, _i, _i, _i, _d, _vp]),
+    "nsof_stage_iterate_x_resample": (_i, [_vp, _i, _vp, _vp, _i, _i, _i, _i, _i, _d, _vp]),
     "nsof_stage_flow_upsample": (_i, [_vp, _i, _vp, _i, _i, _vp, _i, _i, _d]),
     "nsof_prof_enable": (_i, [_vp, C.c_uint]),
     "nsof_prof_collect": (_i, [_vp, _i, C.POINTER(_d), C.POINTER(C.c_longlong)]),
```
